# videosegmentation/video_segment

Hardware: AMD Instinct MI355X
Metric: over-segmented frames/sec at 1080p (higher is better)
Workload: dtype f32

## Files before the change

### include/vsg.h

```cpp
#ifndef VSG_H_
#define VSG_H_

#include <stddef.h>
#include <stdint.h>

#ifdef __cplusplus
extern "C" {
#endif

#define VSG_OK 0
#define VSG_ERR_INVALID -1
#define VSG_ERR_DEVICE -2
#define VSG_ERR_STATE -3
#define VSG_ERR_INTERNAL -4

#define VSG_MEM_HOST 0
#define VSG_MEM_DEVICE 1

typedef struct vsg_stream vsg_stream;
typedef struct vsg_graph vsg_graph;

typedef struct vsg_options {
  int presmoothing;
  float frac_min_region_size;
  int chunk_size;
  float chunk_overlap_ratio;
  int num_constraint_frames;
  int enforce_n4_connectivity;
  int enforce_spatial_connectedness;
  int color_distance;
  int device;
  int two_stage_oversegment;
  int compute_vectorization;
} vsg_options;

typedef struct vsg_timings {
  float preprocess_ms;
  float edges_ms;
  float sort_ms;
  float merge_ms;
  float readout_ms;
  float host_post_ms;
  int64_t edges_total;
  int64_t edges_active;
  int64_t merges;
  int64_t preprocess_launches;
  int64_t edge_launches;
  float wave_kernel_ms;
  int64_t wave_kernel_launches;
  int64_t wave_kernel_edges;
  float filter_kernel_ms;
  int64_t filter_kernel_launches;
  float spine_kernel_ms;
  int64_t spine_kernel_launches;
  int64_t spine_kernel_edges;
} vsg_timings;

typedef struct vsg_diagnostics {
  double segment_wall_ms;
  double prepare_ms;
  double constrained_merge_ms;
  int64_t stages;
  int64_t optimistic_stages, rollbacks;
  int64_t slab_growths;
  double slab_growth_ms;
  int64_t spine_pool_growths;
  double spine_pool_growth_ms;
  int64_t runtime_mallocs;
  double runtime_malloc_ms;
  int64_t runtime_frees;
  double runtime_free_ms;
  int64_t cache_hits;
  int64_t device_syncs;
  double device_sync_ms;
  int64_t mail_waits;
  double mail_wait_ms;
  double mail_wait_longest_ms;
  int mail_mode;
} vsg_diagnostics;

typedef struct vsg_merge_paths {
  int64_t hub_stages;
  int64_t hub_absorbed;
  int64_t hub_cuts;
  int64_t hub_cuts_in_groups;
  int64_t hub_parts_in_later_bucket;
  int64_t spine_side_cuts;
  int64_t hub_retries;
  int64_t hub_reasons[6];
  int64_t hub_exclusion_reruns;
  int64_t hub_off_reruns;
  int64_t group_halvings;
  int64_t conservative_replays;
} vsg_merge_paths;

typedef struct vsg_spine_paths {
  int64_t replays;
  int64_t components;
  int64_t nested_replays;
  int64_t deepest_level;
  int64_t forest_rounds;
  int64_t forest_rounds_ahead;
  int64_t forest_compactions_ahead;
  int64_t forest_compactions_sync;
  int64_t forest_lists_refused;
  int64_t ranked_by_sampling;
  int64_t ranked_plain;
  int64_t rank_sampling_refused;
  int64_t jump_loops_ended_early;
  int64_t streamed_passes;
  int64_t streamed_refused;
  int64_t pool_fallbacks[4];
  int64_t top_level_fallbacks;
  int64_t nested_fallbacks;
  int64_t assumption_reruns;
  int64_t limit_bucket_moves;
  int64_t low_bucket_failures[2];
  int64_t low_bucket_skips[2];
  int64_t zero_pool_flips;
  int64_t windows_run;
  int64_t rle_stages;
  int64_t wide_launches;
  int64_t group_stages;
  int64_t sorts_hand;
  int64_t sorts_library;
} vsg_spine_paths;

typedef struct vsg_boundary_paths {
  int64_t halo_planes_in_pool;
} vsg_boundary_paths;

typedef struct vsg_memory_stats {
  int64_t bytes_in_use;
  int64_t bytes_in_use_peak;
  int64_t bytes_cached;
  int64_t limit_bytes;
  int64_t runtime_mallocs, runtime_frees, cache_hits, device_syncs;
  double runtime_malloc_ms, runtime_free_ms, device_sync_ms;
} vsg_memory_stats;
int vsg_device_memory_stats(int device, vsg_memory_stats* out);
int vsg_device_memory_trim(int device);
int vsg_device_memory_limit(int device, int64_t bytes);

const char* vsg_last_error(void);
int vsg_version(void);
void vsg_default_options(vsg_options* o);
int vsg_device_count(void);

int vsg_vectorize_id_image(const int32_t* ids, int width, int height, const uint8_t** data,
                           size_t* len);

int vsg_stream_create(const vsg_options* o, int width, int height, vsg_stream** out);
void vsg_stream_destroy(vsg_stream* s);
int vsg_stream_process_frame(vsg_stream* s, int flush, const uint8_t* bgr, size_t stride,
                             const float* flow, int has_flow_stream, int mem, int* num_results);
int vsg_stream_chunk_size(const vsg_stream* s);
int vsg_stream_result_bytes(vsg_stream* s, int i, const uint8_t** data, size_t* len);
int vsg_stream_result_id_image(vsg_stream* s, int i, int32_t* out);
int vsg_stream_last_merge_stats(const vsg_stream* s, int64_t* forced_regular_small);
int vsg_stream_keep_node_states(vsg_stream* s, int on);
int vsg_stream_last_node_states(const vsg_stream* s, int64_t* n, const int32_t** root, const float** mean,
                                const int32_t** size, const int32_t** constraint, const uint8_t** flags);
int vsg_stream_last_timings(const vsg_stream* s, vsg_timings* t);
int vsg_stream_last_diagnostics(const vsg_stream* s, vsg_diagnostics* d);
int vsg_stream_last_merge_paths(const vsg_stream* s, vsg_merge_paths* out);
int vsg_stream_last_spine_paths(const vsg_stream* s, vsg_spine_paths* out);
int vsg_stream_last_boundary_paths(const vsg_stream* s, vsg_boundary_paths* out);
int vsg_stream_last_smoothed(vsg_stream* s, float* out);

int vsg_stream_export_halo(vsg_stream* s, const int32_t** dev_labels_virtual,
                           const int32_t** dev_labels_constrained, int64_t scalars[4]);
int vsg_stream_import_halo(vsg_stream* s, const int32_t* labels_virtual,
                           const int32_t* labels_constrained, int mem, const int64_t scalars[4]);

int vsg_stream_expect_halo(vsg_stream* s);
int vsg_stream_restart(vsg_stream* s);

typedef struct vsg_chain vsg_chain;
int vsg_chain_create(int rank, int world, const char* id_file, uint64_t nonce, int device,
                     vsg_chain** out);
void vsg_chain_destroy(vsg_chain* c);
int vsg_chain_info(const vsg_chain* c, int* rank, int* world);
int vsg_chain_send_halo(vsg_chain* c, vsg_stream* from, int dst);
int vsg_chain_recv_halo(vsg_chain* c, vsg_stream* into, int src);
int vsg_chain_exchange_halo(vsg_chain* c, vsg_stream* from, int dst, vsg_stream* into, int src);

typedef struct vsg_regionseg vsg_regionseg;
typedef struct vsg_regionseg_options {
  int min_region_num;
  int max_region_num;
  float level_cutoff_fraction;
  float small_region_penalizer;
  int luminance_bins;
  int color_bins;
  int flow_bins;
  int chunk_set_size;
  int chunk_set_overlap;
  int constraint_chunks;
  int use_appearance;
  int use_flow;
  int use_size_penalizer;
  int compute_vectorization;
  int save_descriptors;
} vsg_regionseg_options;
void vsg_regionseg_default_options(vsg_regionseg_options* o);
int vsg_regionseg_create(const vsg_regionseg_options* o, int width, int height, vsg_regionseg** out);
void vsg_regionseg_destroy(vsg_regionseg* r);
int vsg_regionseg_process_frame(vsg_regionseg* r, int flush, const uint8_t* seg_desc, size_t seg_len,
                             const uint8_t* bgr, size_t stride, const float* flow, int* num_results);
int vsg_regionseg_result_bytes(vsg_regionseg* r, int i, const uint8_t** data, size_t* len);
int vsg_bgr_to_lab(const uint8_t* bgr, size_t stride, int width, int height, uint8_t* lab);

int vsg_graph_create(int width, int height, int max_frames, int l1, int device, vsg_graph** out);
void vsg_graph_destroy(vsg_graph* g);
int vsg_graph_add_frame_bgr(vsg_graph* g, const uint8_t* bgr, size_t stride, int presmoothing,
                            const int32_t* constraint_ids, int mem);
int vsg_graph_add_frame_features(vsg_graph* g, const float* feat, const int32_t* constraint_ids,
                                 int mem);
int vsg_graph_add_virtual_frame(vsg_graph* g, const int32_t* constraint_ids, int mem);
int vsg_graph_add_temporal(vsg_graph* g, const float* flow, int is_virtual, int mem);
int vsg_graph_finish_building(vsg_graph* g);
int vsg_graph_segment_spatially(vsg_graph* g);
int vsg_graph_segment(vsg_graph* g, int min_region_size, int force_constraints);
int vsg_graph_obtain_results(vsg_graph* g, int use_flows, int enforce_n4,
                             int enforce_spatial_connectedness);
int vsg_graph_num_frames(const vsg_graph* g);
int vsg_graph_num_regions(const vsg_graph* g);
int64_t vsg_graph_num_neighbor_links(const vsg_graph* g);
int vsg_graph_region_sizes(const vsg_graph* g, int32_t* sizes, int32_t* constrained_ids);
int vsg_graph_index_image(const vsg_graph* g, int t, int32_t* out);
typedef struct vsg_region {
  int32_t index, size, constrained_id, first_frame, last_frame;
} vsg_region;
typedef struct vsg_interval {
  int32_t region_index, y, left_x, right_x;
} vsg_interval;
int vsg_graph_get_regions(vsg_graph* g, const vsg_region** regions, size_t* num_regions,
                          const int32_t** nbr_csr_ptr, const int32_t** nbr_csr_idx);
int vsg_graph_get_intervals(vsg_graph* g, int frame, const vsg_interval** intervals, size_t* n);
int vsg_graph_smoothed(vsg_graph* g, int t, float* out );
int vsg_graph_spatial_buckets(vsg_graph* g, int t, uint16_t* out );
int vsg_graph_temporal_buckets(vsg_graph* g, int t, uint16_t* out , int32_t* prev_idx);
int vsg_graph_node_roots(vsg_graph* g, int32_t* out);
int vsg_graph_node_states(vsg_graph* g, int32_t* root, float* mean, int32_t* size, int32_t* constraint,
                          uint8_t* flags);
int vsg_graph_merge_stats(const vsg_graph* g, int64_t* forced_regular_small);
int vsg_graph_timings(const vsg_graph* g, vsg_timings* t);
int vsg_graph_diagnostics(const vsg_graph* g, vsg_diagnostics* d);
int vsg_graph_merge_paths(const vsg_graph* g, vsg_merge_paths* out);
int vsg_graph_spine_paths(const vsg_graph* g, vsg_spine_paths* out);

int vsg_debug_sort_pairs(const uint32_t* keys, const uint32_t* values, int n, int end_bit,
                         uint32_t* keys_out, uint32_t* values_out, int device);
int vsg_debug_sort_pairs_timed(const uint32_t* keys, const uint32_t* values, int n, int end_bit,
                               uint32_t* keys_out, uint32_t* values_out, int device, int impl, int reps,
                               double* avg_us);
int vsg_debug_exclusive_sum(const int32_t* in, int n, int32_t* out, int64_t* total);
int vsg_debug_runs_of_sorted_keys(const uint32_t* keys, int n, int32_t* seg_off, int32_t* seg_cnt,
                                  int32_t* num_runs);

#ifdef __cplusplus
}
#endif
#endif
```

### video_segment_amd/_lib.py

```python
import ctypes as C
import os
import subprocess

_HERE = os.path.dirname(os.path.abspath(__file__))
CSRC_DIR = os.path.join(_HERE, "csrc")
LIB_PATH = os.path.join(_HERE, "lib", "libvsg_hip.so")

VSG_OK = 0
VSG_ERR_INVALID, VSG_ERR_DEVICE, VSG_ERR_STATE, VSG_ERR_INTERNAL = -1, -2, -3, -4
VSG_MEM_HOST = 0
VSG_MEM_DEVICE = 1


class VsgOptions(C.Structure):
    _fields_ = [
        ("presmoothing", C.c_int),
        ("frac_min_region_size", C.c_float),
        ("chunk_size", C.c_int),
        ("chunk_overlap_ratio", C.c_float),
        ("num_constraint_frames", C.c_int),
        ("enforce_n4_connectivity", C.c_int),
        ("enforce_spatial_connectedness", C.c_int),
        ("color_distance", C.c_int),
        ("device", C.c_int),
        ("two_stage_oversegment", C.c_int),
        ("compute_vectorization", C.c_int),
    ]


class VsgTimings(C.Structure):
    _fields_ = [
        ("preprocess_ms", C.c_float),
        ("edges_ms", C.c_float),
        ("sort_ms", C.c_float),
        ("merge_ms", C.c_float),
        ("readout_ms", C.c_float),
        ("host_post_ms", C.c_float),
        ("edges_total", C.c_int64),
        ("edges_active", C.c_int64),
        ("merges", C.c_int64),
        ("preprocess_launches", C.c_int64),
        ("edge_launches", C.c_int64),
        ("wave_kernel_ms", C.c_float),
        ("wave_kernel_launches", C.c_int64),
        ("wave_kernel_edges", C.c_int64),
        ("filter_kernel_ms", C.c_float),
        ("filter_kernel_launches", C.c_int64),
        ("spine_kernel_ms", C.c_float),
        ("spine_kernel_launches", C.c_int64),
        ("spine_kernel_edges", C.c_int64),
    ]


class VsgDiagnostics(C.Structure):
    _fields_ = [
        ("segment_wall_ms", C.c_double), ("prepare_ms", C.c_double), ("constrained_merge_ms", C.c_double),
        ("stages", C.c_int64), ("optimistic_stages", C.c_int64), ("rollbacks", C.c_int64),
        ("slab_growths", C.c_int64), ("slab_growth_ms", C.c_double),
        ("spine_pool_growths", C.c_int64), ("spine_pool_growth_ms", C.c_double),
        ("runtime_mallocs", C.c_int64), ("runtime_malloc_ms", C.c_double),
        ("runtime_frees", C.c_int64), ("runtime_free_ms", C.c_double),
        ("cache_hits", C.c_int64), ("device_syncs", C.c_int64), ("device_sync_ms", C.c_double),
        ("mail_waits", C.c_int64), ("mail_wait_ms", C.c_double), ("mail_wait_longest_ms", C.c_double),
        ("mail_mode", C.c_int),
    ]

    def as_dict(self):
        return {k: getattr(self, k) for k, _ in self._fields_}


class VsgMergePaths(C.Structure):
    _fields_ = [
        ("hub_stages", C.c_int64), ("hub_absorbed", C.c_int64),
        ("hub_cuts", C.c_int64), ("hub_cuts_in_groups", C.c_int64), ("hub_parts_in_later_bucket", C.c_int64),
        ("spine_side_cuts", C.c_int64),
        ("hub_retries", C.c_int64), ("hub_reasons", C.c_int64 * 6),
        ("hub_exclusion_reruns", C.c_int64), ("hub_off_reruns", C.c_int64),
        ("group_halvings", C.c_int64), ("conservative_replays", C.c_int64),
    ]

    def as_dict(self):
        return {k: (list(getattr(self, k)) if k == "hub_reasons" else getattr(self, k)) for k, _ in self._fields_}


class VsgSpinePaths(C.Structure):
    _fields_ = [
        ("replays", C.c_int64), ("components", C.c_int64), ("nested_replays", C.c_int64),
        ("deepest_level", C.c_int64),
        ("forest_rounds", C.c_int64), ("forest_rounds_ahead", C.c_int64), ("forest_compactions_ahead", C.c_int64),
        ("forest_compactions_sync", C.c_int64), ("forest_lists_refused", C.c_int64),
        ("ranked_by_sampling", C.c_int64), ("ranked_plain", C.c_int64), ("rank_sampling_refused", C.c_int64),
        ("jump_loops_ended_early", C.c_int64), ("streamed_passes", C.c_int64), ("streamed_refused", C.c_int64),
        ("pool_fallbacks", C.c_int64 * 4), ("top_level_fallbacks", C.c_int64), ("nested_fallbacks", C.c_int64),
        ("assumption_reruns", C.c_int64), ("limit_bucket_moves", C.c_int64),
        ("low_bucket_failures", C.c_int64 * 2), ("low_bucket_skips", C.c_int64 * 2),
        ("zero_pool_flips", C.c_int64),
        ("windows_run", C.c_int64), ("rle_stages", C.c_int64), ("wide_launches", C.c_int64),
        ("group_stages", C.c_int64), ("sorts_hand", C.c_int64), ("sorts_library", C.c_int64),
    ]

    def as_dict(self):
        return {k: (list(getattr(self, k)) if issubclass(t, C.Array) else getattr(self, k)) for k, t in self._fields_}


class VsgBoundaryPaths(C.Structure):
    _fields_ = [
        ("halo_planes_in_pool", C.c_int64),
    ]

    def as_dict(self):
        return {k: getattr(self, k) for k, _ in self._fields_}


class VsgMemoryStats(C.Structure):
    _fields_ = [
        ("bytes_in_use", C.c_int64), ("bytes_in_use_peak", C.c_int64), ("bytes_cached", C.c_int64),
        ("limit_bytes", C.c_int64),
        ("runtime_mallocs", C.c_int64), ("runtime_frees", C.c_int64), ("cache_hits", C.c_int64),
        ("device_syncs", C.c_int64),
        ("runtime_malloc_ms", C.c_double), ("runtime_free_ms", C.c_double), ("device_sync_ms", C.c_double),
    ]

    def as_dict(self):
        return {k: getattr(self, k) for k, _ in self._fields_}


class VsgRegionOptions(C.Structure):
    _fields_ = [
        ("min_region_num", C.c_int), ("max_region_num", C.c_int),
        ("level_cutoff_fraction", C.c_float), ("small_region_penalizer", C.c_float),
        ("luminance_bins", C.c_int), ("color_bins", C.c_int), ("flow_bins", C.c_int),
        ("chunk_set_size", C.c_int), ("chunk_set_overlap", C.c_int), ("constraint_chunks", C.c_int),
        ("use_appearance", C.c_int), ("use_flow", C.c_int), ("use_size_penalizer", C.c_int),
        ("compute_vectorization", C.c_int), ("save_descriptors", C.c_int),
    ]


EXPORTED_SYMBOLS = [
    "vsg_last_error", "vsg_version", "vsg_default_options", "vsg_device_count",
    "vsg_device_memory_stats", "vsg_device_memory_trim", "vsg_device_memory_limit",
    "vsg_vectorize_id_image",
    "vsg_stream_create", "vsg_stream_destroy", "vsg_stream_process_frame", "vsg_stream_chunk_size",
    "vsg_stream_result_bytes", "vsg_stream_result_id_image", "vsg_stream_last_merge_stats",
    "vsg_stream_keep_node_states", "vsg_stream_last_node_states",
    "vsg_stream_last_timings", "vsg_stream_last_diagnostics", "vsg_stream_last_merge_paths", "vsg_stream_last_spine_paths",
    "vsg_stream_last_boundary_paths",
    "vsg_stream_last_smoothed", "vsg_stream_export_halo",
    "vsg_stream_import_halo", "vsg_stream_expect_halo", "vsg_stream_restart",
    "vsg_chain_create", "vsg_chain_destroy", "vsg_chain_info", "vsg_chain_send_halo",
    "vsg_chain_recv_halo", "vsg_chain_exchange_halo",
    "vsg_regionseg_default_options", "vsg_regionseg_create", "vsg_regionseg_destroy", "vsg_regionseg_process_frame",
    "vsg_regionseg_result_bytes", "vsg_bgr_to_lab",
    "vsg_graph_create", "vsg_graph_destroy", "vsg_graph_add_frame_bgr",
    "vsg_graph_add_frame_features", "vsg_graph_add_virtual_frame", "vsg_graph_add_temporal",
    "vsg_graph_finish_building", "vsg_graph_segment_spatially", "vsg_graph_segment", "vsg_graph_obtain_results",
    "vsg_graph_num_frames", "vsg_graph_num_regions", "vsg_graph_num_neighbor_links",
    "vsg_graph_region_sizes", "vsg_graph_index_image", "vsg_graph_get_regions",
    "vsg_graph_get_intervals", "vsg_graph_smoothed",
    "vsg_graph_spatial_buckets", "vsg_graph_temporal_buckets", "vsg_graph_node_roots",
    "vsg_graph_node_states",
    "vsg_graph_merge_stats", "vsg_graph_timings", "vsg_graph_diagnostics", "vsg_graph_merge_paths",
    "vsg_graph_spine_paths",
    "vsg_debug_sort_pairs", "vsg_debug_sort_pairs_timed", "vsg_debug_exclusive_sum", "vsg_debug_runs_of_sorted_keys",
]


def build(force=False):
    subprocess.check_call(["make", "-C", CSRC_DIR, "-j8", "-s"])
    return LIB_PATH


_lib = None


def lib():
    global _lib
    if _lib is not None:
        return _lib
    if not os.path.exists(LIB_PATH):
        raise RuntimeError(
            "libvsg_hip.so is missing (%s): build the HIP extension first; there is no fallback "
            "path" % LIB_PATH)
    try:
        import torch
    except ImportError:
        pass
    L = C.CDLL(LIB_PATH)
    vp = C.c_void_p
    L.vsg_last_error.restype = C.c_char_p
    L.vsg_version.restype = C.c_int
    L.vsg_default_options.argtypes = [C.POINTER(VsgOptions)]
    L.vsg_device_count.restype = C.c_int
    L.vsg_device_memory_stats.argtypes = [C.c_int, C.POINTER(VsgMemoryStats)]
    L.vsg_device_memory_trim.argtypes = [C.c_int]
    L.vsg_device_memory_limit.argtypes = [C.c_int, C.c_int64]
    L.vsg_vectorize_id_image.argtypes = [vp, C.c_int, C.c_int, C.POINTER(vp), C.POINTER(C.c_size_t)]
    L.vsg_stream_create.argtypes = [C.POINTER(VsgOptions), C.c_int, C.c_int, C.POINTER(vp)]
    L.vsg_stream_destroy.argtypes = [vp]
    L.vsg_stream_process_frame.argtypes = [vp, C.c_int, vp, C.c_size_t, vp, C.c_int, C.c_int,
                                           C.POINTER(C.c_int)]
    L.vsg_stream_chunk_size.argtypes = [vp]
    L.vsg_stream_result_bytes.argtypes = [vp, C.c_int, C.POINTER(vp), C.POINTER(C.c_size_t)]
    L.vsg_stream_result_id_image.argtypes = [vp, C.c_int, vp]
    L.vsg_stream_last_merge_stats.argtypes = [vp, vp]
    L.vsg_stream_keep_node_states.argtypes = [vp, C.c_int]
    L.vsg_stream_last_node_states.argtypes = [vp, C.POINTER(C.c_int64)] + [C.POINTER(vp)] * 5
    L.vsg_stream_last_timings.argtypes = [vp, C.POINTER(VsgTimings)]
    L.vsg_stream_last_diagnostics.argtypes = [vp, C.POINTER(VsgDiagnostics)]
    L.vsg_stream_last_merge_paths.argtypes = [vp, C.POINTER(VsgMergePaths)]
    L.vsg_stream_last_spine_paths.argtypes = [vp, C.POINTER(VsgSpinePaths)]
    L.vsg_stream_last_boundary_paths.argtypes = [vp, C.POINTER(VsgBoundaryPaths)]
    L.vsg_stream_last_smoothed.argtypes = [vp, vp]
    L.vsg_stream_export_halo.argtypes = [vp, C.POINTER(vp), C.POINTER(vp), vp]
    L.vsg_stream_import_halo.argtypes = [vp, vp, vp, C.c_int, vp]
    L.vsg_stream_expect_halo.argtypes = [vp]
    L.vsg_stream_restart.argtypes = [vp]
    L.vsg_chain_create.argtypes = [C.c_int, C.c_int, C.c_char_p, C.c_uint64, C.c_int, C.POINTER(vp)]
    L.vsg_chain_info.argtypes = [vp, C.POINTER(C.c_int), C.POINTER(C.c_int)]
    L.vsg_chain_exchange_halo.argtypes = [vp, vp, C.c_int, vp, C.c_int]
    L.vsg_chain_destroy.argtypes = [vp]
    L.vsg_chain_send_halo.argtypes = [vp, vp, C.c_int]
    L.vsg_chain_recv_halo.argtypes = [vp, vp, C.c_int]
    L.vsg_regionseg_default_options.argtypes = [C.POINTER(VsgRegionOptions)]
    L.vsg_regionseg_create.argtypes = [C.POINTER(VsgRegionOptions), C.c_int, C.c_int, C.POINTER(vp)]
    L.vsg_regionseg_destroy.argtypes = [vp]
    L.vsg_regionseg_process_frame.argtypes = [vp, C.c_int, vp, C.c_size_t, vp, C.c_size_t, vp, C.POINTER(C.c_int)]
    L.vsg_regionseg_result_bytes.argtypes = [vp, C.c_int, C.POINTER(vp), C.POINTER(C.c_size_t)]
    L.vsg_bgr_to_lab.argtypes = [vp, C.c_size_t, C.c_int, C.c_int, vp]
    L.vsg_debug_sort_pairs.argtypes = [vp, vp, C.c_int, C.c_int, vp, vp, C.c_int]
    L.vsg_debug_sort_pairs_timed.argtypes = [vp, vp, C.c_int, C.c_int, vp, vp, C.c_int, C.c_int, C.c_int,
                                             C.POINTER(C.c_double)]
    L.vsg_graph_create.argtypes = [C.c_int, C.c_int, C.c_int, C.c_int, C.c_int, C.POINTER(vp)]
    L.vsg_graph_destroy.argtypes = [vp]
    L.vsg_graph_add_frame_bgr.argtypes = [vp, vp, C.c_size_t, C.c_int, vp, C.c_int]
    L.vsg_graph_add_frame_features.argtypes = [vp, vp, vp, C.c_int]
    L.vsg_graph_add_virtual_frame.argtypes = [vp, vp, C.c_int]
    L.vsg_graph_add_temporal.argtypes = [vp, vp, C.c_int, C.c_int]
    L.vsg_graph_finish_building.argtypes = [vp]
    L.vsg_graph_segment_spatially.argtypes = [vp]
    L.vsg_graph_segment.argtypes = [vp, C.c_int, C.c_int]
    L.vsg_graph_obtain_results.argtypes = [vp, C.c_int, C.c_int, C.c_int]
    L.vsg_graph_num_frames.argtypes = [vp]
    L.vsg_graph_num_regions.argtypes = [vp]
    L.vsg_graph_num_neighbor_links.argtypes = [vp]
    L.vsg_graph_num_neighbor_links.restype = C.c_int64
    L.vsg_graph_region_sizes.argtypes = [vp, vp, vp]
    L.vsg_graph_index_image.argtypes = [vp, C.c_int, vp]
    L.vsg_graph_get_regions.argtypes = [vp, C.POINTER(vp), C.POINTER(C.c_size_t), C.POINTER(vp),
                                        C.POINTER(vp)]
    L.vsg_graph_get_intervals.argtypes = [vp, C.c_int, C.POINTER(vp), C.POINTER(C.c_size_t)]
    L.vsg_graph_smoothed.argtypes = [vp, C.c_int, vp]
    L.vsg_graph_spatial_buckets.argtypes = [vp, C.c_int, vp]
    L.vsg_graph_temporal_buckets.argtypes = [vp, C.c_int, vp, vp]
    L.vsg_graph_node_roots.argtypes = [vp, vp]
    L.vsg_graph_node_states.argtypes = [vp, vp, vp, vp, vp, vp]
    L.vsg_graph_merge_stats.argtypes = [vp, vp]
    L.vsg_graph_timings.argtypes = [vp, C.POINTER(VsgTimings)]
    L.vsg_graph_diagnostics.argtypes = [vp, C.POINTER(VsgDiagnostics)]
    L.vsg_graph_merge_paths.argtypes = [vp, C.POINTER(VsgMergePaths)]
    L.vsg_graph_spine_paths.argtypes = [vp, C.POINTER(VsgSpinePaths)]
    L.vsg_debug_exclusive_sum.argtypes = [vp, C.c_int, vp, C.POINTER(C.c_int64)]
    L.vsg_debug_runs_of_sorted_keys.argtypes = [vp, C.c_int, vp, vp, C.POINTER(C.c_int32)]
    _lib = L
    return L


class VsgError(RuntimeError):

    def __init__(self, msg, code=None):
        super().__init__(msg)
        self.code = code


def memory_stats(device=-1):
    st = VsgMemoryStats()
    check(lib().vsg_device_memory_stats(device, C.byref(st)))
    return st.as_dict()


def memory_trim(device=-1):
    check(lib().vsg_device_memory_trim(device))


def memory_limit(nbytes, device=-1):
    check(lib().vsg_device_memory_limit(device, int(nbytes)))


def check(rc):
    if rc != VSG_OK:
        raise VsgError("vsg error %d: %s" % (rc, lib().vsg_last_error().decode()), rc)
```

### video_segment_amd/csrc/capi.cpp

```cpp
#include <algorithm>
#include <cstring>
#include <memory>
#include <string>
#include <vector>

#include <rccl/rccl.h>

#include <chrono>
#include <cstdio>
#include <fstream>
#include <thread>

#include "../../include/vsg.h"
#include "region_segmentation.h"
#include "scan_device.h"
#include "stream.h"

namespace {

thread_local std::string g_last_error;

template <class F>
int Guard(F&& f) {
  try {
// ... 235 lines not shown
        runs.emplace_back(row[x], vsg::Interval{y, x, x2});
        x = x2 + 1;
      }
    }
    std::stable_sort(runs.begin(), runs.end(),
                     [](const std::pair<int32_t, vsg::Interval>& a,
                        const std::pair<int32_t, vsg::Interval>& b) { return a.first < b.first; });
    vsg::SegDesc d;
    d.frame_width = width;
    d.frame_height = height;
    for (const auto& r : runs) {
      if (d.regions.empty() || d.regions.back().id != r.first) {
        d.regions.emplace_back();
        d.regions.back().id = r.first;
      }
      d.regions.back().raster.push_back(r.second);
    }
    for (auto& r : d.regions) vsg::MomentsFromRaster(r.raster, &r.moments);
    vsg::ComputeFrameVectorization(&d);
    wire = vsg::EncodeSegDesc(d);
    *data = reinterpret_cast<const uint8_t*>(wire.data());
    *len = wire.size();
  });
}

static void RequireFrameSize(int width, int height) {
  VSG_REQUIRE(width >= 2 && width <= vsg::kMaxFrameWidth && height >= 1 && height <= vsg::kMaxFrameHeight,
              VSG_ERR_INVALID,
              "unsupported frame size " + std::to_string(width) + "x" + std::to_string(height) +
                  ": width has to be in [2, " + std::to_string(vsg::kMaxFrameWidth) +
                  "], height in [1, " + std::to_string(vsg::kMaxFrameHeight) + "]");
}

int vsg_stream_create(const vsg_options* o, int width, int height, vsg_stream** out) {
  return Guard([&] {
    VSG_REQUIRE(o && out, VSG_ERR_INVALID, "null argument");
    RequireFrameSize(width, height);
    RequireDevice(o->device);
    std::unique_ptr<vsg_stream> s(new vsg_stream);
    s->device = ResolveDevice(o->device);
    DeviceGuard dg(s->device);
    vsg_options opts = *o;
    opts.device = s->device;
    s->impl.reset(new vsg::DenseSegmentationHip(opts, width, height));
    *out = s.release();
  });
}

void vsg_stream_destroy(vsg_stream* s) {
  if (!s) return;
  (void)Guard([&] {
    DeviceGuard dg(s->device);
    s->impl.reset();
  });
  delete s;
}

int vsg_stream_process_frame(vsg_stream* s, int flush, const uint8_t* bgr, size_t stride,
                             const float* flow, int has_flow_stream, int mem, int* num_results) {
  return Guard([&] {
    VSG_REQUIRE(s && num_results, VSG_ERR_INVALID, "null argument");
    DeviceGuard dg(s->device);
    *num_results = s->impl->ProcessFrame(flush != 0, bgr, stride, flow, has_flow_stream != 0, mem);
  });
}

int vsg_stream_chunk_size(const vsg_stream* s) { return s ? s->impl->ChunkSize() : VSG_ERR_INVALID; }

int vsg_stream_result_bytes(vsg_stream* s, int i, const uint8_t** data, size_t* len) {
  return Guard([&] {
    VSG_REQUIRE(s && data && len, VSG_ERR_INVALID, "null argument");
    DeviceGuard dg(s->device);
    VSG_REQUIRE(i >= 0 && i < s->impl->num_results(), VSG_ERR_INVALID, "result index");
    const std::string& b = s->impl->result_bytes(i);
    *data = reinterpret_cast<const uint8_t*>(b.data());
    *len = b.size();
  });
}

int vsg_stream_result_id_image(vsg_stream* s, int i, int32_t* out) {
  return Guard([&] {
    VSG_REQUIRE(s && out, VSG_ERR_INVALID, "null argument");
    DeviceGuard dg(s->device);
    VSG_REQUIRE(i >= 0 && i < s->impl->num_results(), VSG_ERR_INVALID, "result index");
    const size_t n = (size_t)s->impl->W() * s->impl->H();
    for (size_t k = 0; k < n; ++k) out[k] = -1;
    vsg::RenderIdImage(s->impl->result(i), s->impl->W(), out);
  });
}

int vsg_stream_last_merge_stats(const vsg_stream* s, int64_t* st) {
  return Guard([&] {
    VSG_REQUIRE(s && st, VSG_ERR_INVALID, "null argument");
    DeviceGuard dg(s->device);
    s->impl->last_merge_stats(st);
  });
}

int vsg_stream_keep_node_states(vsg_stream* s, int on) {
  return Guard([&] {
    VSG_REQUIRE(s, VSG_ERR_INVALID, "null argument");
    s->impl->keep_node_states(on != 0);
  });
}

int vsg_stream_last_node_states(const vsg_stream* s, int64_t* n, const int32_t** root, const float** mean,
                                const int32_t** size, const int32_t** constraint, const uint8_t** flags) {
  return Guard([&] {
    VSG_REQUIRE(s && n && root && mean && size && constraint && flags, VSG_ERR_INVALID, "null argument");
    const auto& st = s->impl->last_node_states();
    VSG_REQUIRE(!st.root.empty(), VSG_ERR_STATE, "no chunk has been segmented with keeping on");
    *n = (int64_t)st.root.size();
    *root = st.root.data();
    *mean = st.mean.data();
    *size = st.size.data();
    *constraint = st.constraint.data();
    *flags = st.flags.data();
  });
}

int vsg_stream_last_timings(const vsg_stream* s, vsg_timings* t) {
  return Guard([&] {
    VSG_REQUIRE(s && t, VSG_ERR_INVALID, "null argument");
    DeviceGuard dg(s->device);
    *t = s->impl->last_timings();
  });
}

int vsg_stream_last_diagnostics(const vsg_stream* s, vsg_diagnostics* d) {
  return Guard([&] {
    VSG_REQUIRE(s && d, VSG_ERR_INVALID, "null argument");
    FillDiagnostics(s->impl->last_graph_timings(), d);
  });
}

int vsg_stream_last_merge_paths(const vsg_stream* s, vsg_merge_paths* out) {
  return Guard([&] {
    VSG_REQUIRE(s && out, VSG_ERR_INVALID, "null argument");
    FillMergePaths(s->impl->last_graph_timings().paths, out);
  });
}

int vsg_stream_last_spine_paths(const vsg_stream* s, vsg_spine_paths* out) {
  return Guard([&] {
    VSG_REQUIRE(s && out, VSG_ERR_INVALID, "null argument");
    FillSpinePaths(s->impl->last_graph_timings().spine_paths, out);
  });
}

int vsg_stream_last_boundary_paths(const vsg_stream* s, vsg_boundary_paths* out) {
  return Guard([&] {
    VSG_REQUIRE(s && out, VSG_ERR_INVALID, "null argument");
    *out = s->impl->last_boundary_paths();
  });
}

int vsg_stream_last_smoothed(vsg_stream* s, float* out) {
  return Guard([&] {
    VSG_REQUIRE(s && out, VSG_ERR_INVALID, "null argument");
    DeviceGuard dg(s->device);
    s->impl->CopyLastSmoothed(out);
  });
}

int vsg_stream_export_halo(vsg_stream* s, const int32_t** virt, const int32_t** cons,
                           int64_t scalars[4]) {
  return Guard([&] {
    VSG_REQUIRE(s && virt && cons && scalars, VSG_ERR_INVALID, "null argument");
    DeviceGuard dg(s->device);
    s->impl->ExportHalo(virt, cons, scalars);
  });
}

int vsg_stream_expect_halo(vsg_stream* s) {
  return Guard([&] {
    VSG_REQUIRE(s, VSG_ERR_INVALID, "null argument");
    DeviceGuard dg(s->device);
    s->impl->ExpectHalo();
  });
}

int vsg_stream_restart(vsg_stream* s) {
  return Guard([&] {
    VSG_REQUIRE(s, VSG_ERR_INVALID, "null argument");
    DeviceGuard dg(s->device);
    s->impl->Restart();
  });
}

int vsg_stream_import_halo(vsg_stream* s, const int32_t* virt, const int32_t* cons, int mem,
                           const int64_t scalars[4]) {
  return Guard([&] {
    VSG_REQUIRE(s && virt && cons && scalars, VSG_ERR_INVALID, "null argument");
    DeviceGuard dg(s->device);
    s->impl->ImportHalo(virt, cons, mem, scalars);
  });
}

}

#define VSG_NCCL(call)                                                                      \
  do {                                                                                      \
    ncclResult_t r_ = (call);                                                               \
    if (r_ != ncclSuccess) {                                                                \
      vsg::Throw(VSG_ERR_DEVICE, std::string("RCCL: ") + ncclGetErrorString(r_) + " in " #call); \
    }                                                                                       \
  } while (0)

struct vsg_chain {
  int rank = 0, world = 1, device = 0;
  ncclComm_t comm = nullptr;
  hipStream_t stream = nullptr;
  vsg::DevBuf<int32_t> send_staging, recv_staging;
};

namespace {

struct ChainIdFile {
  char magic[8];
  uint64_t nonce;
  ncclUniqueId id;
};
const char kChainMagic[8] = {'V', 'S', 'G', 'C', 'H', 'A', 'I', 'N'};

}

extern "C" {

int vsg_chain_create(int rank, int world, const char* id_file, uint64_t nonce, int device,
                     vsg_chain** out) {
  return Guard([&] {
    VSG_REQUIRE(out && id_file && world >= 1 && rank >= 0 && rank < world, VSG_ERR_INVALID,
                "bad argument");
    RequireDevice(device);
    std::unique_ptr<vsg_chain> c(new vsg_chain);
    c->rank = rank;
    c->world = world;
    c->device = ResolveDevice(device);
    DeviceGuard dg(c->device);
    ChainIdFile rec;
    const std::string path(id_file);
    if (rank == 0) {
      (void)std::remove(path.c_str());
      std::memcpy(rec.magic, kChainMagic, sizeof(rec.magic));
      rec.nonce = nonce;
      VSG_NCCL(ncclGetUniqueId(&rec.id));
      const std::string tmp = path + ".tmp";
      {
        std::ofstream f(tmp.c_str(), std::ios::binary | std::ios::trunc);
        f.write(reinterpret_cast<const char*>(&rec), sizeof(rec));
        VSG_REQUIRE(f.good(), VSG_ERR_INVALID, "cannot write the communicator id file");
      }
      VSG_REQUIRE(std::rename(tmp.c_str(), path.c_str()) == 0, VSG_ERR_INVALID,
                  "cannot publish the communicator id file");
    } else {
      bool got = false;
      for (int attempt = 0; attempt < 1200 && !got; ++attempt) {
        std::ifstream f(path.c_str(), std::ios::binary);
        if (f.good()) {
          f.read(reinterpret_cast<char*>(&rec), sizeof(rec));
          got = f.gcount() == (std::streamsize)sizeof(rec) &&
                std::memcmp(rec.magic, kChainMagic, sizeof(rec.magic)) == 0 && rec.nonce == nonce;
        }
        if (!got) std::this_thread::sleep_for(std::chrono::milliseconds(100));
      }
      VSG_REQUIRE(got, VSG_ERR_STATE,
                  "timed out waiting for the communicator id file of this run (nonce mismatch or "
                  "rank 0 never started)");
    }
    VSG_NCCL(ncclCommInitRank(&c->comm, world, rec.id, rank));
    if (rank == 0) (void)std::remove(path.c_str());
    VSG_HIP(hipStreamCreateWithFlags(&c->stream, hipStreamNonBlocking));
    *out = c.release();
  });
}

void vsg_chain_destroy(vsg_chain* c) {
  if (!c) return;
  (void)Guard([&] {
    DeviceGuard dg(c->device);
    if (c->stream) (void)hipStreamSynchronize(c->stream);
    if (c->comm) (void)ncclCommDestroy(c->comm);
    if (c->stream) (void)hipStreamDestroy(c->stream);
    c->send_staging.release();
    c->recv_staging.release();
  });
  delete c;
}

int vsg_chain_info(const vsg_chain* c, int* rank, int* world) {
  return Guard([&] {
    VSG_REQUIRE(c && rank && world, VSG_ERR_INVALID, "null argument");
    DeviceGuard dg(c->device);
    VSG_NCCL(ncclCommUserRank(c->comm, rank));
    VSG_NCCL(ncclCommCount(c->comm, world));
  });
}

int vsg_chain_exchange_halo(vsg_chain* c, vsg_stream* from, int dst, vsg_stream* into, int src) {
  return Guard([&] {
    VSG_REQUIRE(c && (from || into), VSG_ERR_INVALID, "bad argument");
    VSG_REQUIRE(!from || (dst >= 0 && dst < c->world), VSG_ERR_INVALID, "destination rank");
    VSG_REQUIRE(!into || (src >= 0 && src < c->world), VSG_ERR_INVALID, "source rank");
    VSG_REQUIRE(!from || dst != c->rank || (into && src == c->rank), VSG_ERR_INVALID,
                "a send to the own rank needs the matching receive in the same call");
    VSG_REQUIRE(!into || src != c->rank || (from && dst == c->rank), VSG_ERR_INVALID,
// ... 156 lines not shown
    if (n == 0) return;
    vsg::DevBuf<uint32_t> k((size_t)n), v((size_t)n), ko((size_t)n), vo((size_t)n);
    vsg::DevBuf<uint8_t> temp(vsg::SortPairsU32TempBytes(n));
    hipStream_t s = nullptr;
    VSG_HIP(hipStreamCreateWithFlags(&s, hipStreamNonBlocking));
    hipEvent_t e0 = nullptr, e1 = nullptr;
    struct Owner {
      hipStream_t& s;
      hipEvent_t &e0, &e1;
      ~Owner() {
        if (e0) (void)hipEventDestroy(e0);
        if (e1) (void)hipEventDestroy(e1);
        (void)hipStreamDestroy(s);
      }
    } owner{s, e0, e1};
    VSG_HIP(hipEventCreate(&e0));
    VSG_HIP(hipEventCreate(&e1));
    VSG_HIP(hipMemcpyAsync(k.get(), keys, (size_t)n * 4, hipMemcpyHostToDevice, s));
    VSG_HIP(hipMemcpyAsync(v.get(), values, (size_t)n * 4, hipMemcpyHostToDevice, s));
    auto sort = impl == 1 ? vsg::SortPairsU32Hand : impl == 2 ? vsg::SortPairsU32Lib : vsg::SortPairsU32;
    sort(temp.get(), temp.size(), k.get(), ko.get(), v.get(), vo.get(), n, end_bit, s);
    VSG_HIP(hipEventRecord(e0, s));
    for (int r = 0; r < reps; ++r) sort(temp.get(), temp.size(), k.get(), ko.get(), v.get(), vo.get(), n, end_bit, s);
    VSG_HIP(hipEventRecord(e1, s));
    VSG_HIP(hipMemcpyAsync(keys_out, ko.get(), (size_t)n * 4, hipMemcpyDeviceToHost, s));
    VSG_HIP(hipMemcpyAsync(values_out, vo.get(), (size_t)n * 4, hipMemcpyDeviceToHost, s));
    VSG_HIP(hipStreamSynchronize(s));
    float ms = 0;
    VSG_HIP(hipEventElapsedTime(&ms, e0, e1));
    if (avg_us) *avg_us = (double)ms * 1e3 / reps;
  });
}

int vsg_debug_sort_pairs(const uint32_t* keys, const uint32_t* values, int n, int end_bit,
                         uint32_t* keys_out, uint32_t* values_out, int device) {
  return vsg_debug_sort_pairs_timed(keys, values, n, end_bit, keys_out, values_out, device, 0, 1, nullptr);
}

namespace {
struct DebugStream {
  hipStream_t s = nullptr;
  DebugStream() { VSG_HIP(hipStreamCreateWithFlags(&s, hipStreamNonBlocking)); }
  ~DebugStream() { (void)hipStreamDestroy(s); }
};
}

int vsg_debug_exclusive_sum(const int32_t* in, int n, int32_t* out, int64_t* total) {
  return Guard([&] {
    VSG_REQUIRE(in && out && total && n >= 0, VSG_ERR_INVALID, "bad argument");
    RequireDevice(-1);
    if (n == 0) return;
    vsg::DevBuf<int32_t> d_in((size_t)n), d_out(in == out ? (size_t)1 : (size_t)n), sums(vsg::kScanMaxTiles), d_total(1);
    int32_t* o = in == out ? d_in.get() : d_out.get();
    DebugStream st;
    VSG_HIP(hipMemcpyAsync(d_in.get(), in, (size_t)n * 4, hipMemcpyHostToDevice, st.s));
    vsg::DebugExclusiveSum(vsg::ScanScratch{sums.get(), nullptr}, d_in.get(), o, n, d_total.get(), st.s);
    int32_t t = 0;
    VSG_HIP(hipMemcpyAsync(out, o, (size_t)n * 4, hipMemcpyDeviceToHost, st.s));
    VSG_HIP(hipMemcpyAsync(&t, d_total.get(), 4, hipMemcpyDeviceToHost, st.s));
    VSG_HIP(hipStreamSynchronize(st.s));
    *total = t;
  });
}

int vsg_debug_runs_of_sorted_keys(const uint32_t* keys, int n, int32_t* seg_off, int32_t* seg_cnt,
                                  int32_t* num_runs) {
  return Guard([&] {
    VSG_REQUIRE(keys && seg_off && seg_cnt && num_runs && n >= 0, VSG_ERR_INVALID, "bad argument");
    RequireDevice(-1);
    if (n == 0) return;
    vsg::DevBuf<uint32_t> d_keys((size_t)n);
    vsg::DevBuf<int32_t> d_off((size_t)n), d_cnt((size_t)n), sums(vsg::kScanMaxTiles), d_runs(1);
    DebugStream st;
    VSG_HIP(hipMemcpyAsync(d_keys.get(), keys, (size_t)n * 4, hipMemcpyHostToDevice, st.s));
    VSG_HIP(hipMemcpyAsync(d_off.get(), seg_off, (size_t)n * 4, hipMemcpyHostToDevice, st.s));
    VSG_HIP(hipMemcpyAsync(d_cnt.get(), seg_cnt, (size_t)n * 4, hipMemcpyHostToDevice, st.s));
    vsg::RunsOfSortedKeys(vsg::ScanScratch{sums.get(), nullptr}, d_keys.get(), n, d_off.get(), d_cnt.get(), d_runs.get(),
                          st.s);
    VSG_HIP(hipMemcpyAsync(seg_off, d_off.get(), (size_t)n * 4, hipMemcpyDeviceToHost, st.s));
    VSG_HIP(hipMemcpyAsync(seg_cnt, d_cnt.get(), (size_t)n * 4, hipMemcpyDeviceToHost, st.s));
    VSG_HIP(hipMemcpyAsync(num_runs, d_runs.get(), 4, hipMemcpyDeviceToHost, st.s));
    VSG_HIP(hipStreamSynchronize(st.s));
  });
}

int vsg_graph_create(int width, int height, int max_frames, int l1, int device, vsg_graph** out) {
  return Guard([&] {
    VSG_REQUIRE(out, VSG_ERR_INVALID, "null argument");
    RequireFrameSize(width, height);
    RequireDevice(device);
    std::unique_ptr<vsg_graph> g(new vsg_graph);
    g->device = ResolveDevice(device);
    DeviceGuard dg(g->device);
    g->W = width;
    g->H = height;
    g->wh = (size_t)width * height;
    VSG_HIP(hipStreamCreateWithFlags(&g->stream, hipStreamNonBlocking));
    g->g.reset(new vsg::DenseGraphHip(width, height, max_frames, l1 != 0, g->stream));
    g->pre.reset(new vsg::Preprocessor(width, height, g->stream));
    std::memset(&g->timings, 0, sizeof(g->timings));
    *out = g.release();
  });
}

void vsg_graph_destroy(vsg_graph* g) {
  if (!g) return;
  (void)Guard([&] {
    DeviceGuard dg(g->device);
    if (g->stream) (void)hipStreamSynchronize(g->stream);
    vsg::QuiesceGuard quiesce;
    quiesce.Begin();
    g->g.reset();
    g->pre.reset();
    g->feats.clear();
    g->staging_bgr.release();
    g->staging_f32.release();
    g->staging_ids.release();
    g->flows_dev.clear();
    if (g->stream) (void)hipStreamDestroy(g->stream);
    g->stream = nullptr;
  });
  delete g;
}

static const int32_t* StageIds(vsg_graph* g, const int32_t* ids, int mem) {
  if (!ids) return nullptr;
  if (mem == VSG_MEM_DEVICE) return ids;
  g->staging_ids.ensure(g->wh);
  VSG_HIP(hipMemcpyAsync(g->staging_ids.get(), ids, g->wh * sizeof(int32_t), hipMemcpyHostToDevice,
                         g->stream));
  return g->staging_ids.get();
}

int vsg_graph_add_frame_bgr(vsg_graph* g, const uint8_t* bgr, size_t stride, int presmoothing,
                            const int32_t* constraint_ids, int mem) {
  return Guard([&] {
    VSG_REQUIRE(g && bgr, VSG_ERR_INVALID, "null argument");
    DeviceGuard dg(g->device);
    VSG_REQUIRE(stride >= (size_t)g->W * 3, VSG_ERR_INVALID, "stride smaller than a row");
    const uint8_t* dev = bgr;
    if (mem == VSG_MEM_HOST) {
      g->staging_bgr.ensure(stride * (size_t)g->H);
      VSG_HIP(hipMemcpyAsync(g->staging_bgr.get(), bgr,
                             stride * (size_t)(g->H - 1) + (size_t)g->W * 3, hipMemcpyHostToDevice,
                             g->stream));
      dev = g->staging_bgr.get();
    }
    auto feat = std::make_shared<vsg::DevBuf<float>>(3 * g->wh);
    g->pre->Run(dev, stride, presmoothing, feat->get());
    g->timings.preprocess_ms += g->pre->last_ms();
    g->timings.preprocess_launches += 1;
    const int32_t* ids = StageIds(g, constraint_ids, mem);
    g->g->AddFrame(feat->get(), ids);
    VSG_HIP(hipStreamSynchronize(g->stream));
    g->feats.push_back(feat);
    g->flows_dev.push_back(nullptr);
  });
}

int vsg_graph_add_frame_features(vsg_graph* g, const float* feat_in, const int32_t* constraint_ids,
                                 int mem) {
  return Guard([&] {
    VSG_REQUIRE(g && feat_in, VSG_ERR_INVALID, "null argument");
    DeviceGuard dg(g->device);
    const float* src = feat_in;
    if (mem == VSG_MEM_HOST) {
      g->staging_f32.ensure(3 * g->wh);
      VSG_HIP(hipMemcpyAsync(g->staging_f32.get(), feat_in, 3 * g->wh * sizeof(float),
                             hipMemcpyHostToDevice, g->stream));
      src = g->staging_f32.get();
    }
    auto feat = std::make_shared<vsg::DevBuf<float>>(3 * g->wh);
    vsg::LaunchInterleavedToPlanar(src, g->wh, feat->get(), g->stream);
    const int32_t* ids = StageIds(g, constraint_ids, mem);
    g->g->AddFrame(feat->get(), ids);
    VSG_HIP(hipStreamSynchronize(g->stream));
    g->feats.push_back(feat);
    g->flows_dev.push_back(nullptr);
  });
}

int vsg_graph_add_virtual_frame(vsg_graph* g, const int32_t* constraint_ids, int mem) {
  return Guard([&] {
    VSG_REQUIRE(g && constraint_ids, VSG_ERR_INVALID, "null argument");
    DeviceGuard dg(g->device);
    std::vector<int32_t> host(g->wh);
    if (mem == VSG_MEM_HOST) {
      std::memcpy(host.data(), constraint_ids, g->wh * sizeof(int32_t));
    } else {
      VSG_HIP(hipMemcpy(host.data(), constraint_ids, g->wh * sizeof(int32_t), hipMemcpyDeviceToHost));
    }
    int max_label = 0;
    for (int32_t v : host) max_label = std::max(max_label, v + 1);
    const int32_t* ids = StageIds(g, constraint_ids, mem);
    g->g->AddVirtualFrame(ids, std::max(max_label, 1));
    VSG_HIP(hipStreamSynchronize(g->stream));
    g->feats.push_back(nullptr);
    g->flows_dev.push_back(nullptr);
  });
}

int vsg_graph_add_temporal(vsg_graph* g, const float* flow, int is_virtual, int mem) {
  return Guard([&] {
    VSG_REQUIRE(g, VSG_ERR_INVALID, "null argument");
    DeviceGuard dg(g->device);
    const int nf = g->g->num_frames();
    VSG_REQUIRE(nf >= 2, VSG_ERR_STATE, "temporal edges need two slices");
    const float* fdev = nullptr;
    if (flow) {
      auto fd = std::make_shared<vsg::DevBuf<float>>(2 * g->wh);
      VSG_HIP(hipMemcpyAsync(fd->get(), flow, 2 * g->wh * sizeof(float),
                             mem == VSG_MEM_HOST ? hipMemcpyHostToDevice : hipMemcpyDeviceToDevice,
                             g->stream));
      g->flows_dev[nf - 1] = fd;
      fdev = fd->get();
    }
    const float* cur = g->feats[nf - 1] ? g->feats[nf - 1]->get() : nullptr;
    const float* prev = g->feats[nf - 2] ? g->feats[nf - 2]->get() : nullptr;
    VSG_REQUIRE(is_virtual || (cur && prev), VSG_ERR_STATE, "real temporal edges need two real slices");
    g->g->AddTemporal(cur, prev, fdev, is_virtual != 0);
    VSG_HIP(hipStreamSynchronize(g->stream));
  });
}

int vsg_graph_finish_building(vsg_graph* g) {
  return Guard([&] {
    VSG_REQUIRE(g, VSG_ERR_INVALID, "null argument");
    DeviceGuard dg(g->device);
    g->g->FinishBuilding();
  });
}

int vsg_graph_segment_spatially(vsg_graph* g) {
  return Guard([&] {
    VSG_REQUIRE(g, VSG_ERR_INVALID, "null argument");
    DeviceGuard dg(g->device);
    g->g->SegmentSpatially();
  });
}

int vsg_graph_segment(vsg_graph* g, int min_region_size, int force_constraints) {
  return Guard([&] {
    VSG_REQUIRE(g, VSG_ERR_INVALID, "null argument");
    DeviceGuard dg(g->device);
    g->g->Segment(min_region_size, force_constraints != 0);
  });
}

int vsg_graph_obtain_results(vsg_graph* g, int use_flows, int enforce_n4,
                             int enforce_spatial_connectedness) {
  return Guard([&] {
    VSG_REQUIRE(g, VSG_ERR_INVALID, "null argument");
    DeviceGuard dg(g->device);
    std::vector<const float*> flows;
    if (use_flows) {
      for (auto& f : g->flows_dev) flows.push_back(f ? f->get() : nullptr);
    }
    g->g->ObtainResults(use_flows ? &flows : nullptr, enforce_n4 != 0,
                        enforce_spatial_connectedness != 0);
  });
}

int vsg_graph_num_frames(const vsg_graph* g) { return g ? g->g->num_frames() : VSG_ERR_INVALID; }
int vsg_graph_num_regions(const vsg_graph* g) {
  return g ? (int)g->g->regions().size() : VSG_ERR_INVALID;
}
int64_t vsg_graph_num_neighbor_links(const vsg_graph* g) {
  if (!g) return VSG_ERR_INVALID;
  int64_t n = 0;
  for (const auto& r : g->g->regions()) n += (int64_t)r.neighbors.size();
  return n;
}

int vsg_graph_region_sizes(const vsg_graph* g, int32_t* sizes, int32_t* constrained_ids) {
  return Guard([&] {
    VSG_REQUIRE(g && sizes && constrained_ids, VSG_ERR_INVALID, "null argument");
    DeviceGuard dg(g->device);
    const auto& regs = g->g->regions();
    for (size_t i = 0; i < regs.size(); ++i) {
      sizes[i] = regs[i].size;
      constrained_ids[i] = regs[i].constrained_id;
    }
  });
}

int vsg_graph_index_image(const vsg_graph* g, int t, int32_t* out) {
  return Guard([&] {
    VSG_REQUIRE(g && out, VSG_ERR_INVALID, "null argument");
    DeviceGuard dg(g->device);
    for (size_t k = 0; k < g->wh; ++k) out[k] = -1;
    for (const auto& r : g->g->regions()) {
      if (!r.has_raster) continue;
      for (const auto& sl : r.raster) {
        if (sl.frame != t) continue;
        for (const auto& iv : sl.raster) {
          for (int x = iv.lx; x <= iv.rx; ++x) out[(size_t)iv.y * g->W + x] = r.index;
        }
      }
    }
  });
}

int vsg_graph_get_regions(vsg_graph* g, const vsg_region** regions, size_t* num_regions,
                          const int32_t** nbr_csr_ptr, const int32_t** nbr_csr_idx) {
  return Guard([&] {
    VSG_REQUIRE(g && regions && num_regions && nbr_csr_ptr && nbr_csr_idx, VSG_ERR_INVALID,
                "null argument");
    const auto& regs = g->g->regions();
    g->out_regions.resize(regs.size());
    g->out_nbr_ptr.assign(regs.size() + 1, 0);
    g->out_nbr_idx.clear();
    for (size_t i = 0; i < regs.size(); ++i) {
      const vsg::RegionInfo& r = regs[i];
      VSG_REQUIRE(r.index == (int)i, VSG_ERR_INTERNAL, "region table out of order");
      vsg_region& o = g->out_regions[i];
      o.index = r.index;
      o.size = r.size;
      o.constrained_id = r.constrained_id;
      const bool has = r.has_raster && !r.raster.empty();
      o.first_frame = has ? r.raster.front().frame : -1;
      o.last_frame = has ? r.raster.back().frame : -1;
      g->out_nbr_idx.insert(g->out_nbr_idx.end(), r.neighbors.begin(), r.neighbors.end());
      g->out_nbr_ptr[i + 1] = (int32_t)g->out_nbr_idx.size();
    }
    if (g->out_nbr_idx.empty()) g->out_nbr_idx.push_back(0);
    *regions = g->out_regions.data();
    *num_regions = regs.size();
    *nbr_csr_ptr = g->out_nbr_ptr.data();
// ... 127 lines not shown
```

### video_segment_amd/csrc/dense_graph.cpp

```cpp
#include "dense_graph.h"
#include "scan_device.h"

#include <algorithm>
#include <chrono>
#include <cmath>
#include <cstring>
#include <atomic>
#include <functional>
#include <thread>
#include <unordered_set>

namespace vsg {

namespace {
template <class T>
DevBuf<T>& Grow(DevBuf<T>& b, size_t n) {
  if (b.size() < n) b.alloc(n + n / 2 + 1024);
  return b;
}
double NowMs() {
  using clk = std::chrono::steady_clock;
  return std::chrono::duration<double, std::milli>(clk::now().time_since_epoch()).count();
}
template <class T>
void D2H(T* dst, const T* src, size_t n, hipStream_t s) {
  if (n == 0) return;
  VSG_HIP(hipMemcpyAsync(dst, src, n * sizeof(T), hipMemcpyDeviceToHost, s));
}
template <class T>
void H2D(T* dst, const T* src, size_t n, hipStream_t s) {
  if (n == 0) return;
  VSG_HIP(hipMemcpyAsync(dst, src, n * sizeof(T), hipMemcpyHostToDevice, s));
}
}

DenseGraphHip::DenseGraphHip(int W, int H, int max_frames, bool l1, hipStream_t stream)
    : W_(W), H_(H), capacity_frames_(max_frames), max_frames_(max_frames), l1_(l1),
      stream_(stream), wh_((size_t)W * H) {
  VSG_REQUIRE(W >= 2 && H >= 1 && W <= kMaxFrameWidth && H <= kMaxFrameHeight, -1, "unsupported frame size");
  VSG_REQUIRE(max_frames >= 1 && max_frames < 4096, -1, "unsupported number of frames");
  const size_t N = wh_ * (size_t)max_frames;
  VSG_REQUIRE(N * 9 < (size_t)0xFFFFFFFFu, -1, "graph too large for 32-bit edge positions");
  parent_.alloc(N);
  desc_sz_.alloc(N);
  cons_.alloc(N);
  flags_.alloc(N);
  hub8_.alloc(N);
  cc_.alloc(N);
  label_uf_.alloc(N);
  label_img_.alloc(N);
  adjust_.alloc(N);
  lists_.resize(2 * max_frames - 1);
  list_desc_dev_.alloc(lists_.size());
  list_slot_base_dev_.alloc(lists_.size() + 1);
  const size_t total_slots = (size_t)(4 * max_frames + 9 * (max_frames - 1)) * wh_;
  kept_all_.alloc(total_slots);
  bucket_base_dev_.alloc((size_t)(kNumBuckets + 1) * (lists_.size() + 1));
  keys_tmp_.alloc(9 * wh_ + 8);
  hist_tmp_.alloc(EdgeSortHistInts(wh_));
  hist_sums_.alloc(EdgeSortSumInts(wh_) + 1);
  scalars_.alloc(32);
  stats_.alloc(96);
  hub_excl_.alloc(kHubListInts);
  VSG_HIP(hipMemsetAsync(hub_excl_.get(), 0, 4 * sizeof(int32_t), stream_));
  {
    const int slots = 256;
    const size_t list_cap = 8192;
    const size_t bytes = (size_t)slots * kMailValues * sizeof(unsigned long long) + list_cap * sizeof(int32_t);
    mail_mem_ = CacheAlloc(bytes, kCacheMappedCoherent);
    std::memset(mail_mem_, 0, bytes);
    void* dev = nullptr;
    VSG_HIP(hipHostGetDevicePointer(&dev, mail_mem_, 0));
    mail_.host = static_cast<volatile unsigned long long*>(mail_mem_);
    mail_.dev = static_cast<unsigned long long*>(dev);
    mail_.slots = slots;
    mail_.list_host = reinterpret_cast<volatile int32_t*>(static_cast<char*>(mail_mem_) +
                                                          (size_t)slots * kMailValues * sizeof(unsigned long long));
    mail_.list_dev = reinterpret_cast<int32_t*>(static_cast<char*>(dev) +
                                                (size_t)slots * kMailValues * sizeof(unsigned long long));
    mail_.list_cap = (int)list_cap;
    zero_pool_mem_.alloc(1 << 20);
    zero_pool_.base = zero_pool_mem_.get();
    zero_pool_.cap = zero_pool_mem_.size();
    if (const char* e = getenv("VSG_ZERO_POOL")) {
      zero_pool_.cap = std::min<size_t>(zero_pool_.cap, std::max<size_t>((size_t)atoll(e), 4096) + kZeroArenaInts);
    }
  }
  VSG_HIP(hipStreamCreateWithFlags(&aux_stream_, hipStreamNonBlocking));
  VSG_HIP(hipStreamCreateWithFlags(&aux2_stream_, hipStreamNonBlocking));
  VSG_HIP(hipEventCreateWithFlags(&aux_fork_, hipEventDisableTiming));
  VSG_HIP(hipEventCreateWithFlags(&aux_join_, hipEventDisableTiming));

  scan_sums_.alloc(kScanMaxTiles);
  Reset(max_frames);
  MailRegisterGraph(1);
}

DenseGraphHip::~DenseGraphHip() {
  quiesce_.Begin();
  MailRegisterGraph(-1);
  for (hipEvent_t e : ev_pool_) (void)hipEventDestroy(e);
  if (aux_fork_) (void)hipEventDestroy(aux_fork_);
  if (aux_join_) (void)hipEventDestroy(aux_join_);
  if (aux_stream_) (void)hipStreamDestroy(aux_stream_);
  if (aux2_stream_) (void)hipStreamDestroy(aux2_stream_);
  if (mail_mem_) CacheFree(mail_mem_);
}

void DenseGraphHip::Reset(int max_frames) {
  VSG_REQUIRE(max_frames >= 1 && max_frames <= capacity_frames_, -1, "max_frames above capacity");
  max_frames_ = max_frames;
  num_frames_ = 0;
  has_constraints_ = false;
  virtual_slices_.clear();
  flattened_ = false;
  spatial_pass_done_ = false;
  halo_pending_ = false;
  deferred_virtual_slice_ = deferred_constrained_slice_ = -1;
  for (auto& lb : lists_) lb.used = false;
  regions_.clear();
  key_to_region_.clear();
  key_size_override_.clear();
  next_region_index_ = 0;
  timings_ = GraphTimings();
}

void DenseGraphHip::ForgetLearned() {
  spine_limit_bucket_ = 0x7fffffff;
  spine_limit_age_ = 0;
  for (int b = 0; b < 2; ++b) {
    spine_low_fails_[b] = spine_low_cooldown_[b] = spine_low_cost_age_[b] = 0;
    spine_low_cost_fail_[b] = spine_low_cost_skip_[b] = 0;
  }
  wave_target_active_ = kNoWindowTarget;
  window_target_.clear();
  hub_bucket_pause_.clear();
  window_target_age_ = 0;
  last_density_ = 1.0;
}

void DenseGraphHip::SortList(ListBuf& lb, int per_px) {
  const int n = (int)(per_px * wh_);
  lb.slots.ensure((size_t)n);
  lb.offsets.ensure(kBucketSlots);
  LaunchBucketSort(keys_tmp_.get(), wh_, per_px, hist_tmp_.get(), hist_sums_.get(),
                   lb.offsets.get(), lb.slots.get(), stream_);
  lb.n = n;
  lb.used = true;
}

void DenseGraphHip::AddFrame(const float* feat, const int32_t* cons_dev) {
  VSG_REQUIRE(num_frames_ < max_frames_, -1, "more frames than max_frames (CHECK_LE)");
  const int t = num_frames_;
  const int base = (int)(wh_ * t);
  LaunchInitNodes(feat, wh_, base, cons_dev, nodes(), stream_);
  ListBuf& lb = lists_[2 * t];
  lb.type = 0;
  lb.base_a = base;
  lb.base_b = base;
  LaunchSpatialKeys(feat, W_, H_, l1_ ? 1 : 0, keys_tmp_.get(), hist_tmp_.get(), stream_);
  SortList(lb, 4);
  if (cons_dev) has_constraints_ = true;
  ++num_frames_;
}

void DenseGraphHip::AddVirtualFrame(const int32_t* ids_dev, int max_label) {
  VSG_REQUIRE(num_frames_ < max_frames_, -1, "more frames than max_frames (CHECK_LE)");
  VSG_REQUIRE(max_label >= 1, -1, "max_label must be positive");
  const int t = num_frames_;
  first_label_scratch_.ensure((size_t)max_label);
  LaunchInitVirtualNodes(ids_dev, wh_, (int)(wh_ * t), max_label, first_label_scratch_.get(),
                         nodes(), stream_);
  virtual_slices_.push_back(t);
  has_constraints_ = true;
  ++num_frames_;
}

void DenseGraphHip::AddVirtualFrameDeferred() {
  VSG_REQUIRE(num_frames_ < max_frames_, -1, "more frames than max_frames (CHECK_LE)");
  deferred_virtual_slice_ = num_frames_;
  deferred_constrained_slice_ = num_frames_ + 1;
  virtual_slices_.push_back(num_frames_);
  has_constraints_ = true;
  halo_pending_ = true;
  ++num_frames_;
}

void DenseGraphHip::SetHaloLabels(const int32_t* virtual_ids_dev, const int32_t* constrained_ids_dev,
                                  int max_label) {
  VSG_REQUIRE(halo_pending_, -3, "no deferred virtual slice");
  VSG_REQUIRE(num_frames_ > deferred_constrained_slice_, -3,
              "the constrained slice has to be added before its labels");
  VSG_REQUIRE(max_label >= 1, -1, "max_label must be positive");
  first_label_scratch_.ensure((size_t)max_label);
  LaunchInitVirtualNodes(virtual_ids_dev, wh_, (int)(wh_ * deferred_virtual_slice_), max_label,
                         first_label_scratch_.get(), nodes(), stream_);
  VSG_HIP(hipMemcpyAsync(cons_.get() + wh_ * (size_t)deferred_constrained_slice_, constrained_ids_dev,
                         wh_ * sizeof(int32_t), hipMemcpyDeviceToDevice, stream_));
  halo_pending_ = false;
}

void DenseGraphHip::AddTemporal(const float* cur, const float* prev, const float* flow,
                                bool is_virtual) {
  VSG_REQUIRE(num_frames_ >= 2, -3, "temporal edges need two slices");
  const int t = num_frames_ - 1;
  ListBuf& lb = lists_[2 * t - 1];
  lb.type = 1;
  lb.base_a = (int)(wh_ * t);
  lb.base_b = (int)(wh_ * (t - 1));
  lb.prev_idx.ensure(wh_);
  LaunchTemporalKeys(cur, prev, flow, W_, H_, l1_ ? 1 : 0, is_virtual ? 1 : 0, keys_tmp_.get(),
                     lb.prev_idx.get(), hist_tmp_.get(), stream_);
  SortList(lb, 9);
}

void DenseGraphHip::FinishBuilding() { VSG_HIP(hipStreamSynchronize(stream_)); }

void DenseGraphHip::EnsureScratch(size_t n) {
  if (n <= scratch_edges_) return;
  n = n + n / 8 + 1024;
  e_ra_.alloc(n);
  e_rb_.alloc(n);
  e_gpos_.alloc(n);
  filter_masks_.alloc(3 * (4 * ((n + 255) / 256) + 4));
  block_cnt_.alloc((n + 255) / 256 + 2);
  block_off_.alloc((n + 255) / 256 + 2);
  scratch_edges_ = n;
}

void DenseGraphHip::EnsureActiveScratch(size_t n) {
  if (n <= scratch_active_) return;
  n = std::max(n + n / 8 + 1024, scratch_active_ + scratch_active_ / 2);
  size_t bytes = 0;
  auto carve = [&bytes](size_t elems, size_t elem_size) {
    const size_t at = bytes;
    bytes += (elems * elem_size + 255) & ~(size_t)255;
    return at;
  };
  const size_t o_e_active = carve(n, 4), o_e_apos = carve(n, 4), o_a_ra = carve(n, 4), o_a_rb = carve(n, 4),
               o_a_gpos = carve(n, 4), o_a_comp = carve(n, 4), o_a_idx = carve(n, 4), o_s_comp = carve(n, 4),
               o_s_idx = carve(n, 4), o_seg_key = carve(n, 4), o_seg_cnt = carve(n, 4), o_seg_off = carve(n, 4),
               o_lead_pos = carve(n, 4), o_l_ra = carve(n, 4), o_l_rb = carve(n, 4), o_l_gpos = carve(n, 4),
               o_bk_ds = carve(2 * n, sizeof(float4)), o_bk_cons = carve(2 * n, 4), o_bk_flags = carve(2 * n, 1);
  scratch_active_ = 0;
  act_ = ActiveArrays();
  active_slab_.alloc(bytes);
  uint8_t* b = active_slab_.get();
  act_.e_active = reinterpret_cast<int32_t*>(b + o_e_active);
  act_.e_apos = reinterpret_cast<int32_t*>(b + o_e_apos);
  act_.a_ra = reinterpret_cast<int32_t*>(b + o_a_ra);
  act_.a_rb = reinterpret_cast<int32_t*>(b + o_a_rb);
  act_.a_gpos = reinterpret_cast<uint32_t*>(b + o_a_gpos);
  act_.a_comp = reinterpret_cast<uint32_t*>(b + o_a_comp);
  act_.a_idx = reinterpret_cast<uint32_t*>(b + o_a_idx);
  act_.s_comp = reinterpret_cast<uint32_t*>(b + o_s_comp);
  act_.s_idx = reinterpret_cast<uint32_t*>(b + o_s_idx);
  act_.seg_key = reinterpret_cast<uint32_t*>(b + o_seg_key);
  act_.seg_cnt = reinterpret_cast<int32_t*>(b + o_seg_cnt);
  act_.seg_off = reinterpret_cast<int32_t*>(b + o_seg_off);
  act_.lead_pos = reinterpret_cast<int32_t*>(b + o_lead_pos);
  act_.l_ra = reinterpret_cast<int32_t*>(b + o_l_ra);
  act_.l_rb = reinterpret_cast<int32_t*>(b + o_l_rb);
  act_.l_gpos = reinterpret_cast<uint32_t*>(b + o_l_gpos);
  act_.bk_ds = reinterpret_cast<float4*>(b + o_bk_ds);
  act_.bk_cons = reinterpret_cast<int32_t*>(b + o_bk_cons);
  act_.bk_flags = b + o_bk_flags;
  const size_t temp = SortPairsU32TempBytes((int)std::min<size_t>(2 * n, 0x7fffffff));
  if (temp > cub_temp_.size()) cub_temp_.alloc(temp);
  scratch_active_ = n;
}

void DenseGraphHip::RunStageDebug(int b, int w, int windows, int j0, int n, const MergeParams& P,
                                  int inert_mode, MergeScratch& S, bool debug_stages, StageInfo* info) {
  unsigned long long s0[96] = {0}, s1[96] = {0};
  double ts = 0;
  size_t ev0 = 0, evf0 = 0;
  if (debug_stages) {
    VSG_HIP(hipMemsetAsync(stats_.get() + 16, 0, 2 * sizeof(unsigned long long), stream_));
    VSG_HIP(hipMemsetAsync(stats_.get() + 48, 0, 16 * sizeof(unsigned long long), stream_));
    D2H(s0, stats_.get(), 96, stream_);
    VSG_HIP(hipStreamSynchronize(stream_));
    ts = NowMs();
    ev0 = ev_wave_.size();
    evf0 = ev_filter_.size();
  }
  RunBucketStage(b, j0, n, list_desc_dev_.get(), bucket_base_dev_.get(), list_slot_base_dev_.get(),
                 kept_all_.get(), nodes(), P, inert_mode, S, stream_, info);
  if (!debug_stages) return;
  D2H(s1, stats_.get(), 96, stream_);
  VSG_HIP(hipStreamSynchronize(stream_));
  const double te = NowMs();
  float wave_ms = 0;
  for (size_t k = ev0; k < ev_wave_.size(); ++k) {
    float ms = 0;
    VSG_HIP(hipEventElapsedTime(&ms, ev_pool_[ev_wave_[k].first], ev_pool_[ev_wave_[k].second]));
    wave_ms += ms;
  }
  float filter_ms = 0;
  for (size_t k = evf0; k < ev_filter_.size(); ++k) {
    float ms = 0;
    VSG_HIP(hipEventElapsedTime(&ms, ev_pool_[ev_filter_[k].first], ev_pool_[ev_filter_[k].second]));
    filter_ms += ms;
  }
  if (te - ts <= 1.0) return;
  std::fprintf(stderr, "[vsg] stage b=%d w=%d/%d n=%d wall %.2f ms filter %.2f ms workers %.2f ms | replayed %d components %d | "
               "wave edges %llu batches %llu rounds %llu nwin %llu chain %llu | max_seg %llu slowest %.2f Mcyc | "
               "cyc load %.0f M loop %.0f M wait %.0f M\n",
               b, w, windows, n, te - ts, filter_ms, wave_ms, info ? info->replayed : -1, info ? info->components : -1,
               s1[3] - s0[3], s1[7] - s0[7], s1[5] - s0[5], s1[4] - s0[4], s1[20] - s0[20],
               s1[17], s1[16] / 1e6, (s1[18] - s0[18]) / 1e6, (s1[19] - s0[19]) / 1e6,
               (s1[26] - s0[26]) / 1e6);
  std::fprintf(stderr, "[vsg]   largest: %.2f Mcyc batches %llu rounds %llu live %llu chain %llu nwin %llu | kcyc/batch: "
               "wait %.1f stage+table %.1f loop %.1f (reserve %.1f closure %.1f masks+generic %.1f chain %.1f) | cuts %llu kept %llu\n",
               s1[48] / 1e6, s1[49], s1[50], s1[51], s1[55], s1[56],
               s1[52] / 1e3 / std::max(1.0, (double)s1[49]), s1[53] / 1e3 / std::max(1.0, (double)s1[49]),
               s1[54] / 1e3 / std::max(1.0, (double)s1[49]), s1[57] / 1e3 / std::max(1.0, (double)s1[49]),
               s1[58] / 1e3 / std::max(1.0, (double)s1[49]), s1[59] / 1e3 / std::max(1.0, (double)s1[49]),
               s1[60] / 1e3 / std::max(1.0, (double)s1[49]), s1[61], s1[62]);
  std::fprintf(stderr, "[vsg]   chain ends (%llu): not owner %llu, flags %llu, constraint %llu, larger %llu, failed/mode %llu, "
               "hot small %llu, none %llu\n", s1[71] - s0[71], s1[64] - s0[64], s1[65] - s0[65], s1[66] - s0[66],
               s1[67] - s0[67], s1[68] - s0[68], s1[69] - s0[69], s1[70] - s0[70]);
}

void DenseGraphHip::SegmentLists(int min_region_size, bool force_constraints, int pass) {
  VSG_REQUIRE(num_frames_ >= 1, -3, "no frames");
  VSG_REQUIRE(!halo_pending_, -3, "the labels of the previous chunk have not been imported");
  min_region_size_ = min_region_size;
  const int L = (int)lists_.size();
  const size_t N = wh_ * (size_t)num_frames_;
  const double t_enter = NowMs();
  const ThreadAllocCounters alloc0 = ThreadAllocSnapshot();
  MailWaitResetLongest();
  const MailWaitCounters mail0 = MailWaitSnapshot();
  int64_t diag_stages = 0, diag_slab_growths = 0, diag_spine_growths = 0, diag_hub_stages = 0, diag_hub_absorbed = 0;
  double diag_slab_ms = 0, diag_spine_ms = 0;

  std::vector<ListDesc> desc(L);
  list_slot_base_.assign(L + 1, 0);
  uint32_t acc = 0;
  int64_t edges_total = 0;
  for (int l = 0; l < L; ++l) {
    ListBuf& lb = lists_[l];
    list_slot_base_[l] = acc;
    ListDesc d = {};
    if (lb.used) {
      d.slots = lb.slots.get();
      d.kept = kept_all_.get() + acc;
      d.prev_idx = lb.type == 1 ? lb.prev_idx.get() : nullptr;
      d.offsets = (pass == 1 && lb.type == 1) ? nullptr : lb.offsets.get();
      d.type = lb.type;
      d.base_a = lb.base_a;
      d.base_b = lb.base_b;
      d.n = lb.n;
      acc += (uint32_t)lb.n;
    }
    desc[l] = d;
  }
  list_slot_base_[L] = acc;
  H2D(list_desc_dev_.get(), desc.data(), (size_t)L, stream_);
  H2D(list_slot_base_dev_.get(), list_slot_base_.data(), (size_t)L + 1, stream_);
  if (pass == 2) {
    kept_spatial_pass_.ensure(kept_all_.size());
    VSG_HIP(hipMemcpyAsync(kept_spatial_pass_.get(), kept_all_.get(), acc, hipMemcpyDeviceToDevice,
                           stream_));
  }
  VSG_HIP(hipMemsetAsync(kept_all_.get(), 0, acc, stream_));
  LaunchBuildBucketTable(list_desc_dev_.get(), L, bucket_base_dev_.get(), stream_);
  bucket_base_host_.resize((size_t)(kNumBuckets + 1) * (L + 1));
  D2H(bucket_base_host_.data(), bucket_base_dev_.get(), bucket_base_host_.size(), stream_);
  VSG_HIP(hipMemsetAsync(stats_.get(), 0, 96 * sizeof(unsigned long long), stream_));
  VSG_HIP(hipMemsetAsync(zero_pool_.base, 0, zero_pool_.cap * sizeof(int32_t), stream_));
  zero_pool_.used = 0;
  zero_pool_.second_half = false;
  zero_pool_.arena_used = 0;
  LaunchInitIdentity(cc_.get(), N, stream_);
  VSG_HIP(hipStreamSynchronize(stream_));

  const bool group_buckets = !getenv("VSG_GROUP_BUCKETS") || atoi(getenv("VSG_GROUP_BUCKETS")) != 0;
  std::vector<int32_t> bucket_prefix(kNumBuckets + 2, 0);
  int first_plain = kNumBuckets;
  {
    const float scale = 2048.0f / (1.0f + 1e-6f);
    const float inv_scale = (float)(1.0 / (double)scale);
    const float force_w = l1_ ? 0.002f : 0.001f;
    for (int b = 0; b < kNumBuckets; ++b) {
      if (!((float)b * inv_scale < force_w)) {
        first_plain = b;
        break;
      }
    }
  }
  int64_t n_max = 0;
  for (int b = 0; b <= kNumBuckets; ++b) {
    const int tot = bucket_base_host_[(size_t)b * (L + 1) + L];
    edges_total += tot;
    bucket_prefix[b + 1] = bucket_prefix[b] + tot;
  }
  for (int b = 0; b < kNumBuckets; ++b) n_max = std::max<int64_t>(n_max, bucket_prefix[b + 1] - bucket_prefix[b]);
  VSG_REQUIRE(bucket_prefix[kNumBuckets] >= 0, -1, "too many edges");
  EnsureScratch((size_t)std::max<int64_t>(n_max, 1));
  if (const char* e = getenv("VSG_ACTIVE_CAP")) {
    EnsureActiveScratch((size_t)std::max(1, atoi(e)));
  } else {
    EnsureActiveScratch(std::min<size_t>((size_t)std::max<int64_t>(n_max, 1),
                                         std::max<size_t>((size_t)n_max / 6, (size_t)1 << 20)));
  }
  bucket_prefix_dev_.ensure(bucket_prefix.size());
  H2D(bucket_prefix_dev_.get(), bucket_prefix.data(), bucket_prefix.size(), stream_);

  MergeScratch S = {};
  auto bind_scratch = [this, &S]() {
    S.e_ra = e_ra_.get();
    S.e_rb = e_rb_.get();
    S.e_gpos = e_gpos_.get();
    S.e_active = act_.e_active;
    S.e_apos = act_.e_apos;
    S.a_ra = act_.a_ra;
    S.a_rb = act_.a_rb;
    S.a_gpos = act_.a_gpos;
    S.a_comp = act_.a_comp;
    S.a_idx = act_.a_idx;
    S.s_comp = act_.s_comp;
    S.s_idx = act_.s_idx;
    S.seg_key = act_.seg_key;
    S.seg_cnt = act_.seg_cnt;
    S.seg_off = act_.seg_off;
    S.lead_pos = act_.lead_pos;
    S.l_ra = act_.l_ra;
    S.l_rb = act_.l_rb;
    S.l_gpos = act_.l_gpos;
    S.bk_ds = act_.bk_ds;
    S.bk_cons = act_.bk_cons;
    S.bk_flags = act_.bk_flags;
    S.cub_temp = cub_temp_.get();
    S.cub_temp_bytes = cub_temp_.size();
    S.scan = ScanScratch{scan_sums_.get(), stream_};
    S.active_cap = (int)std::min<size_t>(scratch_active_, 0x7fffffff);
  };
  bind_scratch();
  S.grow_active = [this, bind_scratch, &diag_slab_growths, &diag_slab_ms](long long need) {
    const double tg0 = NowMs();
    VSG_HIP(hipStreamSynchronize(stream_));
    VSG_HIP(hipStreamSynchronize(aux_stream_));
    VSG_HIP(hipStreamSynchronize(aux2_stream_));
    const size_t before = scratch_active_;
    EnsureActiveScratch((size_t)need);
    bind_scratch();
    ++diag_slab_growths;
    diag_slab_ms += NowMs() - tg0;
    if (getenv("VSG_DEBUG_STATS")) {
      std::fprintf(stderr, "[vsg] stage scratch: %zu -> %zu active edges (needed %lld), %.2f ms\n", before,
                   scratch_active_, need, NowMs() - tg0);
    }
    return true;
  };
  S.num_active = scalars_.get();
  S.num_segs = scalars_.get() + 1;
  S.node_key_bits = 1;
  while (S.node_key_bits < 32 && ((size_t)1 << S.node_key_bits) < N) ++S.node_key_bits;
  {
    const size_t words = 4 * ((scratch_edges_ + 255) / 256) + 4;
    S.masks.active = filter_masks_.get();
    S.masks.settled = filter_masks_.get() + words;
    S.masks.tentative = filter_masks_.get() + 2 * words;
    S.masks.block_cnt = block_cnt_.get();
    S.block_off = block_off_.get();
  }
  S.force_rollback = getenv("VSG_FORCE_ROLLBACK") ? 1 : 0;
  S.small_seg = getenv("VSG_SMALL_SEG") ? std::max(1, atoi(getenv("VSG_SMALL_SEG"))) : 24;
  S.wide_min = getenv("VSG_WIDE_MIN") ? atoi(getenv("VSG_WIDE_MIN")) : 0;
  S.wide_waves = getenv("VSG_WIDE_WAVES") ? atoi(getenv("VSG_WIDE_WAVES")) : 4;
  S.chain_relax = getenv("VSG_CHAIN_RELAX") ? atoi(getenv("VSG_CHAIN_RELAX")) : 1;
  const int hubs_default = getenv("VSG_HUBS") ? atoi(getenv("VSG_HUBS")) : 1;
  S.hubs = hubs_default;
  S.hub_excl = hub_excl_.get();
  S.hub_max_splits = getenv("VSG_HUB_SPLITS") ? std::max(0, atoi(getenv("VSG_HUB_SPLITS"))) : kHubMaxSplits;
  S.hub_cut_min_work = getenv("VSG_CUT_MIN_WORK") ? atoi(getenv("VSG_CUT_MIN_WORK")) : 0;
  S.hub_cut_ratio = getenv("VSG_CUT_RATIO") ? std::max(0, atoi(getenv("VSG_CUT_RATIO"))) : 1500;
  S.hub_check = (getenv("VSG_HUB_CHECK") && atoi(getenv("VSG_HUB_CHECK")) != 0) ? 1 : 0;
// ... 1101 lines not shown
          idx = next_region_index_++;
          key_to_region_.emplace(rep_key, idx);
          regions_.emplace_back();
          regions_.back().index = idx;
          regions_.back().size = sz[0];
          regions_.back().constrained_id = cons[0];
        } else {
          idx = it->second;
        }
        if (idx != r && idx > r && idx < num_regions) dirty[idx] = 1;
        regions_[idx].has_raster = true;
        regions_[idx].raster.swap(tr.tubes[k]);
      }
    }
  }

  for (const auto& kv : size_adjust) {
    auto it = key_to_region_.find(kv.first);
    if (it == key_to_region_.end()) {
      key_size_override_[kv.first] = 0;
      continue;
    }
    regions_[it->second].size += kv.second;
  }
  const double t_host1 = NowMs();

  const int n_rl = (int)rl_ty.size();
  if (n_rl > 0) {
    DevBuf<uint32_t>& d_ty = Grow(rl_ty_, n_rl);
    DevBuf<int32_t>&d_lx = Grow(rl_lx_, n_rl), &d_rx = Grow(rl_rx_, n_rl), &d_nl = Grow(rl_nl_, n_rl);
    H2D(d_ty.get(), rl_ty.data(), (size_t)n_rl, stream_);
    H2D(d_lx.get(), rl_lx.data(), (size_t)n_rl, stream_);
    H2D(d_rx.get(), rl_rx.data(), (size_t)n_rl, stream_);
    H2D(d_nl.get(), rl_new.data(), (size_t)n_rl, stream_);
    LaunchRelabelIntervals(d_ty.get(), d_lx.get(), d_rx.get(), d_nl.get(), n_rl, W_, H_,
                           label_uf_.get(), stream_);
    VSG_HIP(hipStreamSynchronize(stream_));
  }
  const int L = (int)lists_.size();
  int capacity = (int)std::max<size_t>(pairs_.size(), (size_t)1 << 20);
  int count = 0;
  bool hashed = false;
  if (!getenv("VSG_PAIR_TABLE") || atoi(getenv("VSG_PAIR_TABLE")) != 0) {
    const size_t cap = (size_t)1 << 21;
    pairs_sorted_.ensure(cap);
    pairs_unique_.ensure(cap);
    pairs_.ensure((size_t)capacity);
    order_keys_.ensure((size_t)capacity);
    PairTable table{pairs_sorted_.get(), pairs_unique_.get(), (unsigned)(cap - 1)};
    LaunchNeighborPairsHashed(list_desc_dev_.get(), L, label_uf_.get(), W_, table, scalars_.get() + 3, stream_);
    int distinct = 0;
    D2H(&distinct, scalars_.get() + 3, 1, stream_);
    VSG_HIP(hipStreamSynchronize(stream_));
    if (distinct <= (int)(cap / 2) && distinct <= capacity) {
      LaunchPairTableCompact(table, pairs_.get(), order_keys_.get(), scalars_.get() + 3, stream_);
      D2H(&count, scalars_.get() + 3, 1, stream_);
      VSG_HIP(hipStreamSynchronize(stream_));
      VSG_REQUIRE(count == distinct, -4, "pair table: entries lost");
      hashed = true;
    }
  }
  for (int attempt = 0; attempt < 2 && !hashed; ++attempt) {
    pairs_.ensure((size_t)capacity);
    order_keys_.ensure((size_t)capacity);
    LaunchNeighborPairs(list_desc_dev_.get(), L, label_uf_.get(), W_, pairs_.get(),
                        order_keys_.get(), scalars_.get() + 3, capacity, stream_);
    D2H(&count, scalars_.get() + 3, 1, stream_);
    VSG_HIP(hipStreamSynchronize(stream_));
    if (count <= capacity) break;
    VSG_REQUIRE(attempt == 0, -4, "neighbour pair buffer overflow");
    capacity = count + 1024;
  }
  std::vector<unsigned long long> uniq;
  if (count > 0) {
    pairs_sorted_.ensure((size_t)count);
    pairs_unique_.ensure((size_t)count);
    size_t temp = std::max(SortKeysU64TempBytes(count), UniqueU64TempBytes(count));
    if (temp > cub_temp_.size()) cub_temp_.alloc(temp);
    SortKeysU64(cub_temp_.get(), cub_temp_.size(), pairs_.get(), pairs_sorted_.get(), count, stream_);
    UniqueU64(cub_temp_.get(), cub_temp_.size(), pairs_sorted_.get(), pairs_unique_.get(),
              scalars_.get() + 4, count, stream_);
    int nu = 0;
    D2H(&nu, scalars_.get() + 4, 1, stream_);
    VSG_HIP(hipStreamSynchronize(stream_));
    uniq.resize(nu);
    D2H(uniq.data(), pairs_unique_.get(), (size_t)nu, stream_);
    VSG_HIP(hipStreamSynchronize(stream_));
  }
  const double t_dev2 = NowMs();

  std::vector<int32_t> unseen;
  for (unsigned long long pr : uniq) {
    const int ka = (int)(uint32_t)(pr >> 32), kb = (int)(uint32_t)(pr & 0xFFFFFFFFull);
    if (!key_to_region_.count(ka)) unseen.push_back(ka);
    if (!key_to_region_.count(kb)) unseen.push_back(kb);
  }
  std::sort(unseen.begin(), unseen.end());
  unseen.erase(std::unique(unseen.begin(), unseen.end()), unseen.end());
  if (!unseen.empty()) {
    const int U = (int)unseen.size();
    DevBuf<int32_t>& d_keys = Grow(un_keys_, U);
    DevBuf<unsigned long long>& d_min = Grow(un_min_, U);
    H2D(d_keys.get(), unseen.data(), (size_t)U, stream_);
    VSG_HIP(hipMemsetAsync(d_min.get(), 0xFF, (size_t)U * sizeof(unsigned long long), stream_));
    LaunchFirstOrderOfKeys(pairs_.get(), order_keys_.get(), count, d_keys.get(), U, d_min.get(),
                           stream_);
    std::vector<unsigned long long> h_min(U);
    D2H(h_min.data(), d_min.get(), (size_t)U, stream_);
    VSG_HIP(hipStreamSynchronize(stream_));
    std::vector<int> order(U);
    for (int i = 0; i < U; ++i) order[i] = i;
    std::sort(order.begin(), order.end(), [&](int a, int b) { return h_min[a] < h_min[b]; });
    std::vector<int32_t> sz, cons;
    fetch_states(unseen, &sz, &cons);
    for (int oi : order) {
      const int key = unseen[oi];
      const int idx = next_region_index_++;
      key_to_region_.emplace(key, idx);
      regions_.emplace_back();
      RegionInfo& ri = regions_.back();
      ri.index = idx;
      auto ov = key_size_override_.find(key);
      ri.size = (ov != key_size_override_.end()) ? ov->second : sz[oi];
      ri.constrained_id = cons[oi];
      ri.has_raster = false;
    }
  }
  for (unsigned long long pr : uniq) {
    const int ka = (int)(uint32_t)(pr >> 32), kb = (int)(uint32_t)(pr & 0xFFFFFFFFull);
    const int ia = key_to_region_.at(ka), ib = key_to_region_.at(kb);
    regions_[ia].neighbors.push_back(ib);
    regions_[ib].neighbors.push_back(ia);
  }
  for (RegionInfo& ri : regions_) {
    std::sort(ri.neighbors.begin(), ri.neighbors.end());
    ri.neighbors.erase(std::unique(ri.neighbors.begin(), ri.neighbors.end()), ri.neighbors.end());
  }
  const double t_end = NowMs();
  if (getenv("VSG_DEBUG_STATS")) {
    std::fprintf(stderr, "[vsg] readout: device1 %.1f host1 %.1f device2 %.1f host2 %.1f ms (intervals %d, pairs %d, unique %zu)\n",
                 t_dev1 - t_start, t_host1 - t_dev1, t_dev2 - t_host1, t_end - t_dev2, num_iv, count,
                 uniq.size());
    std::fprintf(stderr, "[vsg]   host1: region table %.1f, tube prepare %.1f, flow samples %.1f, tube finish %.1f, "
                 "bookkeeping %.1f ms (%zu regions, %lld matched tubes, at most %d in a region)\n", th[0] - t_dev1,
                 th[1] - th[0], th[2] - th[1], th[3] - th[2], t_host1 - th[3], regions_.size(), sum_tubes, most_tubes);
  }
  timings_.readout_ms = (float)((t_dev1 - t_start) + (t_dev2 - t_host1));
  timings_.host_post_ms = (float)((t_host1 - t_dev1) + (t_end - t_dev2));
}

void DenseGraphHip::CopySpatialBuckets(int t, uint16_t* out) {
  VSG_REQUIRE(t >= 0 && t < num_frames_ && lists_[2 * t].used, -1, "no spatial list for slice");
  ListBuf& lb = lists_[2 * t];
  std::vector<uint32_t> slots(lb.n);
  std::vector<int32_t> offs(kBucketSlots);
  D2H(slots.data(), lb.slots.get(), (size_t)lb.n, stream_);
  D2H(offs.data(), lb.offsets.get(), (size_t)kBucketSlots, stream_);
  VSG_HIP(hipStreamSynchronize(stream_));
  for (size_t i = 0; i < 4 * wh_; ++i) out[i] = 0xFFFF;
  for (int b = 0; b <= kNumBuckets; ++b) {
    for (int p = offs[b]; p < offs[b + 1]; ++p) {
      const uint32_t s = slots[p];
      out[(size_t)(s & 3u) * wh_ + (s >> 2)] = (uint16_t)b;
    }
  }
}

void DenseGraphHip::CopyTemporalBuckets(int t, uint16_t* out, int32_t* prev_idx) {
  VSG_REQUIRE(t >= 1 && t < num_frames_ && lists_[2 * t - 1].used, -1, "no temporal list");
  ListBuf& lb = lists_[2 * t - 1];
  std::vector<uint32_t> slots(lb.n);
  std::vector<int32_t> offs(kBucketSlots);
  D2H(slots.data(), lb.slots.get(), (size_t)lb.n, stream_);
  D2H(offs.data(), lb.offsets.get(), (size_t)kBucketSlots, stream_);
  D2H(prev_idx, lb.prev_idx.get(), wh_, stream_);
  VSG_HIP(hipStreamSynchronize(stream_));
  for (size_t i = 0; i < 9 * wh_; ++i) out[i] = 0xFFFF;
  for (int b = 0; b <= kNumBuckets; ++b) {
    for (int p = offs[b]; p < offs[b + 1]; ++p) {
      const uint32_t s = slots[p];
      const uint32_t pix = s / 9u, k = s - pix * 9u;
      out[(size_t)k * wh_ + pix] = (uint16_t)b;
    }
  }
}

void DenseGraphHip::CopyNodeRoots(int32_t* out) {
  const size_t N = wh_ * (size_t)num_frames_;
  LaunchFlatten(nodes(), N, label_uf_.get(), stream_);
  D2H(out, label_uf_.get(), N, stream_);
  VSG_HIP(hipStreamSynchronize(stream_));
}

void DenseGraphHip::CopyNodeStates(int32_t* root, float* mean, int32_t* size, int32_t* cons,
                                   uint8_t* flags) {
  const size_t N = wh_ * (size_t)num_frames_;
  if (N == 0) return;
  DevBuf<int32_t> d_root(N), d_cons(N), d_flags(N);
  DevBuf<float4> d_ds(N);
  std::vector<float4> h_ds(N);
  std::vector<int32_t> h_flags(N);
  LaunchFlatten(nodes(), N, d_root.get(), stream_);
  LaunchGatherStates(nodes(), d_root.get(), (int)N, d_ds.get(), d_cons.get(), d_flags.get(), stream_);
  D2H(root, d_root.get(), N, stream_);
  D2H(h_ds.data(), d_ds.get(), N, stream_);
  D2H(cons, d_cons.get(), N, stream_);
  D2H(h_flags.data(), d_flags.get(), N, stream_);
  VSG_HIP(hipStreamSynchronize(stream_));
  for (size_t i = 0; i < N; ++i) {
    mean[3 * i + 0] = h_ds[i].x;
    mean[3 * i + 1] = h_ds[i].y;
    mean[3 * i + 2] = h_ds[i].z;
    std::memcpy(&size[i], &h_ds[i].w, sizeof(int32_t));
    flags[i] = (uint8_t)h_flags[i];
  }
}

}
```

### video_segment_amd/csrc/dense_graph.h

```cpp
#ifndef VSG_DENSE_GRAPH_H_
#define VSG_DENSE_GRAPH_H_

#include <memory>
#include <unordered_map>
#include <vector>

#include "device_graph.h"
#include "host_model.h"

namespace vsg {

struct MergePaths {
  int64_t hub_stages = 0, hub_absorbed = 0;
  int64_t hub_cuts = 0, hub_cuts_in_groups = 0, hub_parts_in_later_bucket = 0, spine_side_cuts = 0;
  int64_t hub_retries = 0, hub_reasons[6] = {0, 0, 0, 0, 0, 0};
  int64_t hub_exclusion_reruns = 0, hub_off_reruns = 0, group_halvings = 0, conservative_replays = 0;
};

struct GraphTimings {
  float edges_ms = 0, sort_ms = 0, merge_ms = 0, readout_ms = 0, host_post_ms = 0;
  int64_t edges_total = 0, edges_active = 0;
  int64_t merges[3] = {0, 0, 0};
  float wave_ms = 0, filter_ms = 0, spine_ms = 0;
  int64_t wave_launches = 0, filter_launches = 0, wave_edges = 0, spine_launches = 0, spine_edges = 0;
  int64_t optimistic_stages = 0, rollbacks = 0;
  int64_t stages = 0;
  int64_t slab_growths = 0, spine_growths = 0;
  double slab_growth_ms = 0, spine_growth_ms = 0;
  int64_t runtime_mallocs = 0, runtime_frees = 0, cache_hits = 0, device_syncs = 0;
  double runtime_malloc_ms = 0, runtime_free_ms = 0, device_sync_ms = 0;
  int64_t mail_waits = 0;
  double mail_wait_ms = 0, mail_wait_longest_ms = 0;
  int mail_mode = 0;
  double segment_wall_ms = 0, prepare_ms = 0, constrained_merge_ms = 0;
  MergePaths paths;
  SpinePaths spine_paths = {};
};

class DenseGraphHip {
 public:
  DenseGraphHip(int W, int H, int max_frames, bool l1, hipStream_t stream);
  ~DenseGraphHip();

  int W() const { return W_; }
  int H() const { return H_; }
  int max_frames() const { return max_frames_; }
  int num_frames() const { return num_frames_; }
  hipStream_t stream() const { return stream_; }
  hipStream_t aux_stream() const { return aux_stream_; }

  void Reset(int max_frames);
  void ForgetLearned();

  void AddFrame(const float* feat_planar_dev, const int32_t* cons_dev);
  void AddVirtualFrame(const int32_t* ids_dev, int max_label);
  void AddVirtualFrameDeferred();
  void SetHaloLabels(const int32_t* virtual_ids_dev, const int32_t* constrained_ids_dev,
                     int max_label);
  bool halo_pending() const { return halo_pending_; }
  void AddTemporal(const float* cur_dev, const float* prev_dev, const float* flow_dev,
                   bool is_virtual);
  void FinishBuilding();
  void Segment(int min_region_size, bool force_constraints) {
    SegmentLists(min_region_size, force_constraints, spatial_pass_done_ ? 2 : 0);
  }
  void SegmentSpatially() {
    SegmentLists(0, false, 1);
    spatial_pass_done_ = true;
  }
  void ObtainResults(const std::vector<const float*>* dev_flows, bool enforce_n4,
                     bool enforce_spatial_connectedness);

  std::vector<RegionInfo>& regions() { return regions_; }
  const std::vector<RegionInfo>& regions() const { return regions_; }
  const GraphTimings& timings() const { return timings_; }

  void CopySpatialBuckets(int t, uint16_t* out_host);
  void CopyTemporalBuckets(int t, uint16_t* out_host, int32_t* prev_idx_host);
  void CopyNodeRoots(int32_t* out_host);
  void CopyNodeStates(int32_t* root, float* mean, int32_t* size, int32_t* cons, uint8_t* flags);

 private:
  struct ListBuf {
    DevBuf<uint32_t> slots;
    DevBuf<int32_t> offsets;
    DevBuf<int32_t> prev_idx;
    DevBuf<uint16_t> keys_dbg;
    int type = 0;
    int n = 0;
    int base_a = 0, base_b = 0;
    bool used = false;
  };

  void EnsureScratch(size_t n_edges_max);
  void EnsureActiveScratch(size_t n_active_max);
  void DebugHash(const char* where);
  void SortList(ListBuf& lb, int per_px);
  void MergeConstrainedHostAssisted();
  NodeArrays nodes() {
    return NodeArrays{parent_.get(), desc_sz_.get(), cons_.get(), flags_.get(), hub8_.get()};
  }

  QuiesceGuard quiesce_;
  int W_, H_, capacity_frames_, max_frames_;
  bool l1_;
  hipStream_t stream_;
  hipStream_t aux_stream_ = nullptr;
  hipStream_t aux2_stream_ = nullptr;
  hipEvent_t aux_fork_ = nullptr, aux_join_ = nullptr;
  int num_frames_ = 0;
  size_t wh_;
  bool has_constraints_ = false;
  std::vector<int> virtual_slices_;
  int min_region_size_ = 0;
  bool flattened_ = false;

  DevBuf<int32_t> parent_;
  DevBuf<float4> desc_sz_;
  DevBuf<int32_t> cons_;
  DevBuf<uint8_t> flags_;
  DevBuf<uint8_t> hub8_;
  DevBuf<int32_t> cc_, label_uf_, label_img_, adjust_;
  std::vector<ListBuf> lists_;
  DevBuf<ListDesc> list_desc_dev_;
  DevBuf<uint32_t> list_slot_base_dev_;
  std::vector<uint32_t> list_slot_base_;
  DevBuf<uint8_t> kept_all_;
  DevBuf<uint8_t> kept_spatial_pass_;
  bool spatial_pass_done_ = false;
  bool halo_pending_ = false;
  int deferred_virtual_slice_ = -1, deferred_constrained_slice_ = -1;
  void SegmentLists(int min_region_size, bool force_constraints, int pass);
  void RunStageDebug(int b, int w, int windows, int j0, int n, const MergeParams& P, int inert_mode,
                     MergeScratch& S, bool debug_stages, StageInfo* info);
  DevBuf<int32_t> bucket_base_dev_;
  std::vector<int32_t> bucket_base_host_;
  DevBuf<uint16_t> keys_tmp_;
  DevBuf<int32_t> hist_tmp_, hist_sums_;
  DevBuf<int32_t> first_label_scratch_;
  DevBuf<int32_t> e_ra_, e_rb_;
  DevBuf<uint32_t> e_gpos_;
  DevBuf<uint8_t> active_slab_;
  struct ActiveArrays {
    int32_t *e_active = nullptr, *e_apos = nullptr, *a_ra = nullptr, *a_rb = nullptr, *seg_cnt = nullptr,
            *seg_off = nullptr, *lead_pos = nullptr, *l_ra = nullptr, *l_rb = nullptr, *bk_cons = nullptr;
    uint32_t *a_gpos = nullptr, *a_comp = nullptr, *a_idx = nullptr, *s_comp = nullptr, *s_idx = nullptr,
             *seg_key = nullptr, *l_gpos = nullptr;
    float4* bk_ds = nullptr;
    uint8_t* bk_flags = nullptr;
  } act_;
  DevBuf<unsigned long long> filter_masks_;
  DevBuf<int32_t> block_cnt_, block_off_;
  int64_t optimistic_stages_ = 0, rollbacks_ = 0;
  DevBuf<int32_t> scalars_;
  DevBuf<int32_t> seg_table_dev_;
  DevBuf<int32_t> hub_excl_;
  PinnedBuf<int32_t> iv_host_;
  std::vector<int32_t> seg_table_host_, list_off_host_;
  size_t stage_ring_used_ = 0;
  PinnedBuf<int32_t> stage_ring_;
  Mailbox mail_;
  void* mail_mem_ = nullptr;
  DevBuf<int32_t> zero_pool_mem_;
  ZeroPool zero_pool_;
  DevBuf<int32_t> bucket_prefix_dev_;
  int spine_limit_bucket_ = 0x7fffffff;
  int spine_limit_age_ = 0;
  int spine_low_fails_[2] = {0, 0}, spine_low_cooldown_[2] = {0, 0};
  double spine_low_cost_fail_[2] = {0, 0}, spine_low_cost_skip_[2] = {0, 0};
  int spine_low_cost_age_[2] = {0, 0};
  DevBuf<int32_t> spine_pool_;
  static constexpr int64_t kNoWindowTarget = 1ll << 40;
  int64_t wave_target_active_ = kNoWindowTarget;
  std::vector<int64_t> window_target_;
  int window_target_age_ = 0;
  std::vector<int> window_last_seg_;
  std::vector<uint8_t> window_frozen_;
  std::vector<uint8_t> window_unpaid_;
  std::vector<int> window_peak_;
  std::vector<int> hub_bucket_stages_, hub_bucket_pause_;
  std::vector<long long> hub_bucket_absorbed_;
  double last_density_ = 1.0;
  int spine_max_edges_grown_ = 0;
  DevBuf<unsigned long long> stats_;
  DevBuf<uint8_t> cub_temp_;
  DevBuf<int32_t> scan_sums_;
  size_t scratch_edges_ = 0;
  size_t scratch_active_ = 0;
  DevBuf<int32_t> flow_req_dev_;
  DevBuf<float2> flow_samples_dev_;
  DevBuf<const float*> flow_ptrs_dev_;
  void SampleFlows(const std::vector<FlowRequest>& req, const std::vector<const float*>& dev_flows,
                   std::vector<float>* samples);
  DevBuf<int32_t> row_counts_, row_offsets_;
  DevBuf<int32_t> iv_label_, iv_lx_, iv_rx_;
  DevBuf<uint32_t> iv_ty_;
  DevBuf<unsigned long long> pairs_, order_keys_, pairs_sorted_, pairs_unique_;
  DevBuf<int32_t> small_i32_a_, small_i32_b_, small_i32_c_;
  DevBuf<float4> small_f4_;
  DevBuf<int32_t> mc_ids_, mc_par_, mc_cons_, mc_fl_, rl_lx_, rl_rx_, rl_nl_, un_keys_;
  DevBuf<float4> mc_ds_;
  DevBuf<uint32_t> rl_ty_;
  DevBuf<unsigned long long> un_min_;
  std::vector<hipEvent_t> ev_pool_;
  std::vector<std::pair<int, int>> ev_wave_, ev_filter_, ev_spine_;
  int ev_used_ = 0;

  std::vector<RegionInfo> regions_;
  std::unordered_map<int, int> key_to_region_;
  std::unordered_map<int, int> key_size_override_;
  int next_region_index_ = 0;
  GraphTimings timings_;
};

}

#endif
```

### video_segment_amd/csrc/device_graph.h

```cpp
#ifndef VSG_DEVICE_GRAPH_H_
#define VSG_DEVICE_GRAPH_H_

#include <functional>

#include "common.h"

namespace vsg {

constexpr uint8_t kFlagFinalized = 1;
constexpr uint8_t kFlagNoDesc = 2;
constexpr uint8_t kFlagTentative = 4;
constexpr uint8_t kFlagHub = 8;
constexpr uint8_t kFlagHubBroken = 16;
constexpr uint8_t kFlagHubExcluded = 32;
constexpr int kHubExclCap = 16384;
constexpr int kHubMaxAttempts = 4;
constexpr int kHubMaxSplits = 64;
constexpr int kHubCutCap = 64;
constexpr int kHubListInts = 4 + kHubExclCap + 3 * kHubCutCap;

struct NodeArrays {
  int32_t* parent;
  float4* desc_sz;
  int32_t* cons;
  uint8_t* flags;
  uint8_t* hub8;
};

struct ListDesc {
  const uint32_t* slots;
  uint8_t* kept;
  const int32_t* prev_idx;
  const int32_t* offsets;
  int32_t type;
  int32_t base_a;
  int32_t base_b;
  int32_t n;
};

struct MergeParams {
  int W, H;
  int num_lists;
  int min_region_size;
  float force_merge_weight;
  float inv_scale;
  float s_lt_005, s_lt_02, s_le_015;
  const uint8_t* spatial_survivors;
};

void UploadSpaceWeights(const float* w49, hipStream_t stream);
void LaunchMinMax(const uint8_t* bgr, size_t stride, int W, int H, int* mm, hipStream_t s);
void LaunchBilateral(const uint8_t* bgr, size_t stride, int W, int H, const float* lut,
                     float scale, float* planes, hipStream_t s);
void LaunchGaussian3(const uint8_t* bgr, size_t stride, int W, int H, float k0, float k1, float* planes,
                     hipStream_t s);
void LaunchConvertPlanar(const uint8_t* bgr, size_t stride, int W, int H, float* planes,
                         hipStream_t s);
void LaunchInterleavedToPlanar(const float* in, size_t n, float* planes, hipStream_t s);
void LaunchPlanarToInterleaved(const float* planes, size_t n, float* out, hipStream_t s);
size_t EdgeSortHistInts(size_t n_px);
size_t EdgeSortSumInts(size_t n_px);
void LaunchSpatialKeys(const float* feat, int W, int H, int l1, uint16_t* keys, int32_t* hist,
                       hipStream_t s);
void LaunchTemporalKeys(const float* cur, const float* prev, const float* flow, int W, int H,
                        int l1, int is_virtual, uint16_t* keys, int32_t* prev_idx, int32_t* hist,
                        hipStream_t s);
void LaunchBucketSort(const uint16_t* keys, size_t n_px, int per_px, int32_t* hist, int32_t* sums,
                      int32_t* offsets, uint32_t* slots_out, hipStream_t s);
void LaunchInitNodes(const float* feat, size_t n, int base, const int32_t* cons_in,
                     NodeArrays nodes, hipStream_t s);
void LaunchInitVirtualNodes(const int32_t* labels, size_t n, int base, int num_labels,
                            int32_t* first_scratch, NodeArrays nodes, hipStream_t s);

constexpr int kScanMaxTiles = 4096;
struct ScanScratch {
  int32_t* sums;
  hipStream_t owner = nullptr;
};

void DebugExclusiveSum(const ScanScratch& sc, const int32_t* in, int32_t* out, int n, int32_t* total, hipStream_t s);

size_t SortPairsU32HandTempBytes(int n);
void SortPairsU32Hand(void* temp, size_t temp_bytes, const uint32_t* keys_in, uint32_t* keys_out,
                      const uint32_t* vals_in, uint32_t* vals_out, int n, int end_bit, hipStream_t s);
size_t SortPairsU32LibTempBytes(int n);
void SortPairsU32Lib(void* temp, size_t temp_bytes, const uint32_t* keys_in, uint32_t* keys_out,
                     const uint32_t* vals_in, uint32_t* vals_out, int n, int end_bit, hipStream_t s);
size_t SortPairsU32TempBytes(int n);
void SortPairsU32(void* temp, size_t temp_bytes, const uint32_t* keys_in, uint32_t* keys_out,
                  const uint32_t* vals_in, uint32_t* vals_out, int n, int end_bit, hipStream_t s);
bool SortPairsU32TakesHand(int n);
size_t SortKeysU64TempBytes(int n);
void SortKeysU64(void* temp, size_t temp_bytes, const unsigned long long* in,
                 unsigned long long* out, int n,
                 hipStream_t s);
size_t UniqueU64TempBytes(int n);
void UniqueU64(void* temp, size_t temp_bytes, const unsigned long long* in,
               unsigned long long* out,
               int32_t* num_out, int n, hipStream_t s);

constexpr int kMailValues = 4;
struct MailSlot {
  unsigned long long* dev;
  volatile unsigned long long* host;
  unsigned seq;
};
struct Mailbox {
  unsigned long long* dev = nullptr;
  volatile unsigned long long* host = nullptr;
  int slots = 0;
  int next = 0;
  unsigned seq = 0;
  int32_t* list_dev = nullptr;
  volatile int32_t* list_host = nullptr;
  int list_cap = 0;
};
inline MailSlot NextMail(Mailbox& m) {
  MailSlot s{m.dev + (size_t)kMailValues * m.next, m.host + (size_t)kMailValues * m.next, ++m.seq};
  m.next = (m.next + 1) % m.slots;
  return s;
}
void MailWait(const MailSlot& slot, int count, int* values, hipStream_t s);
void MailRegisterGraph(int delta);
int MailYieldMode();
struct MailWaitCounters {
  long long waits = 0;
  double wait_ms = 0, longest_ms = 0;
};
MailWaitCounters MailWaitSnapshot();
void MailWaitResetLongest();
void LaunchMailPost(const MailSlot& slot, const int32_t* p0, const int32_t* p1, const int32_t* p2,
                    const int32_t* p3, hipStream_t s);

constexpr size_t kZeroArenaInts = 1024;
struct ZeroPool {
  int32_t* base = nullptr;
  size_t cap = 0, used = 0;
  bool second_half = false;
  size_t arena_used = 0;
};

struct FilterMasks {
  unsigned long long* active;
  unsigned long long* settled;
  unsigned long long* tentative;
  int32_t* block_cnt;
};
struct FilterSegRec {
  const uint32_t* slots;
  const int32_t* prev;
  int32_t start, pos0, type, base_a, base_b;
  uint32_t slot_base;
};
constexpr int kFilterArgSegs = 64;
struct FilterSegArgs {
  FilterSegRec r[kFilterArgSegs];
};
struct FilterSegs {
  const FilterSegRec* rec;
  int n;
};
constexpr size_t kStageRingInts = (size_t)1 << 18;
struct SpinePaths {
  int64_t replays, components, nested_replays, deepest_level;
  int64_t forest_rounds, forest_rounds_ahead, forest_compactions_ahead, forest_compactions_sync, forest_lists_refused;
  int64_t ranked_by_sampling, ranked_plain, rank_sampling_refused;
  int64_t jump_loops_ended_early, streamed_passes, streamed_refused;
  int64_t pool_fallbacks[4], top_level_fallbacks, nested_fallbacks;
  int64_t assumption_reruns, limit_bucket_moves, low_bucket_failures[2], low_bucket_skips[2];
  int64_t zero_pool_flips;
  int64_t windows_run, rle_stages, wide_launches, group_stages, sorts_hand, sorts_library;
};
struct MergeScratch {
  int active_cap;
  std::function<bool(long long need)> grow_active;
  int32_t* e_ra;
  int32_t* e_rb;
  uint32_t* e_gpos;
  int32_t* e_active;
  int32_t* e_apos;
  FilterMasks masks;
  int32_t* block_off;
  int32_t* a_ra;
  int32_t* a_rb;
  uint32_t* a_gpos;
  uint32_t* a_comp;
  uint32_t* a_idx;
  uint32_t* s_comp;
  uint32_t* s_idx;
  uint32_t* seg_key;
  int32_t* seg_cnt;
  int32_t* seg_off;
  int32_t* num_active;
  int32_t* num_segs;
  float4* bk_ds;
  int32_t* bk_cons;
  uint8_t* bk_flags;
  int force_rollback;
  int32_t* lead_pos;
  int32_t* l_ra;
  int32_t* l_rb;
  uint32_t* l_gpos;
  int use_rle;
  int group_hi;
  const int32_t* bucket_prefix;
  const int32_t* bucket_prefix_host;
  const int32_t* bucket_base_host;
  const int32_t* list_off_host;
  int32_t* seg_dev;
  size_t seg_cap;
  std::vector<int32_t>* seg_host;
  const ListDesc* lists_host;
  int filter_segs_mode;
  int32_t* ring_host;
  size_t ring_cap, *ring_used;
  int spine_min;
  int spine_off;
  int* spine_low_failed;
  const int* spine_low_skip;
  int* spine_limit_bucket;
  int spine_nested_factor;
  int spine_max_edges;
  int spine_debug, spine_check;
  int rank_split_min;
  int spine_fast;
  int spine_fast_min;
  int32_t* spine_pool;
  size_t spine_pool_ints;
  std::function<bool(long long edges)> grow_spine_pool;
  int32_t* nmap[3];
  hipStream_t aux_stream;
  hipStream_t aux2_stream;
  hipEvent_t aux_fork, aux_join;
  int small_seg;
  int wide_min;
  int wide_waves;
  int chain_relax;
  int hubs;
  int hubs_off;
  int hub_attempt;
  int hub_splits_left;
  int hub_split_depth;
  int hub_list_dirty;
  int hub_max_splits;
  int hub_cut_min_work;
  long long hub_splits;
  const uint32_t* list_slot_base_host;
  int32_t* hub_excl;
  long long hub_retries;
  long long hub_reasons[6];
  long long hub_cuts_in_groups;
  long long hub_parts_in_later_bucket;
  long long spine_side_cuts;
  long long hub_exclusion_reruns;
  long long hub_off_reruns;
  long long group_halvings;
  long long conservative_replays;
  long long hub_cut_ratio;
  int hub_check;
  SpinePaths sp;
  int wave_debug;
  int wave_dbg;
  int64_t* optimistic_stages;
  int64_t* rollbacks;
  int32_t* cc;
  unsigned long long* stats;
  void* cub_temp;
  size_t cub_temp_bytes;
  ScanScratch scan;
  int node_key_bits;
  std::vector<hipEvent_t>* ev_pool;
  std::vector<std::pair<int, int>>* ev_wave;
  std::vector<std::pair<int, int>>* ev_filter;
  std::vector<std::pair<int, int>>* ev_spine;
  int* ev_used;
  Mailbox* mail;
  ZeroPool* zeros;
  hipStream_t main_stream;
};
int32_t* TakeZeroed(MergeScratch& S, size_t n);

int32_t* TakeStageScalars(MergeScratch& S, size_t n);

int32_t* TakeStageRing(MergeScratch& S, size_t n);

void LaunchBuildBucketTable(const ListDesc* lists, int num_lists, int32_t* bucket_base,
                            hipStream_t s);
void LaunchInitIdentity(int32_t* a, size_t n, hipStream_t s);
struct StageInfo {
  int want_components = 0;
  int replayed = 0;
  int components = 0;
  int max_wave_segment = 0;
  int hub_stages = 0;
  long long hub_absorbed = 0;
  int hub_retries = 0;
};
void ResetHubExclusions(MergeScratch& S, NodeArrays nodes, hipStream_t s);
void RunBucketStage(int bucket, int j0, int n_b, const ListDesc* lists, const int32_t* bucket_base,
                    const uint32_t* list_slot_base, uint8_t* kept_all, NodeArrays nodes,
                    const MergeParams& P, int inert_mode, MergeScratch& S, hipStream_t s,
                    StageInfo* info = nullptr);
size_t SpinePoolInts(size_t max_edges);
void LaunchKeepVirtualBucket(const ListDesc* lists, int num_lists, hipStream_t s);

void LaunchFlatten(NodeArrays nodes, size_t n, int32_t* label_uf, hipStream_t s);
void LaunchEnforceN4(int32_t* label_img, int W, int H, const int32_t* frames_dev, int num_frames,
                     int32_t* row_flags , int32_t* adjust ,
                     hipStream_t s);
void LaunchRowRunCounts(const int32_t* label_img, int W, int H, const int32_t* frames_dev, int num_frames,
                        int32_t* row_counts , hipStream_t s);
struct IntervalArrays {
  int32_t* label;
  uint32_t* ty;
  int32_t* lx;
  int32_t* rx;
};
void LaunchWriteIntervals(const int32_t* label_img, int W, int H, const int32_t* frames_dev, int num_frames,
                          const int32_t* row_offsets ,
                          IntervalArrays out, hipStream_t s);
void LaunchRelabelIntervals(const uint32_t* ty, const int32_t* lx, const int32_t* rx,
                            const int32_t* new_label, int n, int W, int H, int32_t* label_uf,
                            hipStream_t s);
struct PairTable {
  unsigned long long* key;
// ... 36 lines not shown
```

### video_segment_amd/csrc/edge_sort.hip

```cpp
#include "merge_common.h"

namespace vsg {

constexpr int kTilePxSpatial = 2048;
constexpr int kTilePxTemporal = 1024;
constexpr int kBinInvalid = kBucketSlots - 1;

__device__ __forceinline__ float ColorDist(float ab, float ag, float ar, float bb, float bg,
                                           float br, int l1) {
  const float d1 = ab - bb, d2 = ag - bg, d3 = ar - br;
  if (l1) {
    return (float)((fabs((double)d1) + fabs((double)d2) + fabs((double)d3)) *
                   (double)(1.0f / 3.0f));
  }
  return sqrtf((d1 * d1 + d2 * d2 + d3 * d3) * (1.0f / 3.0f));
}

__device__ __forceinline__ uint16_t BucketOf(float w) {
  const float scale = 2048.0f / (1.0f + 1e-6f);
  return (uint16_t)(int)fminf(2048.0f, w * scale);
}

__device__ __forceinline__ int TruncToIntX86(float v) {
  if (!(v < 2147483648.0f && v >= -2147483648.0f)) return (int)0x80000000;
// ... 107 lines not shown
        }
      }
    }
    __syncthreads();
    const int px_here = (int)min((size_t)256, n - pix0);
    const int words = (px_here * 9 + 1) / 2;
    uint32_t* out32 = reinterpret_cast<uint32_t*>(keys + pix0 * 9);
    const uint32_t* in32 = reinterpret_cast<const uint32_t*>(stage);
    if ((px_here * 9) & 1) {
      for (int w = threadIdx.x; w < words - 1; w += 256) out32[w] = in32[w];
      if (threadIdx.x == 0) keys[pix0 * 9 + (size_t)px_here * 9 - 1] = stage[px_here * 9 - 1];
    } else {
      for (int w = threadIdx.x; w < words; w += 256) out32[w] = in32[w];
    }
    __syncthreads();
  }
  StoreTileHist(lds_hist, blockIdx.x, num_tiles, hist);
}

constexpr int kScanPerBlock = 2048;

__device__ __forceinline__ int BlockExclusiveScan256(int v, int32_t* lds4, int& total) {
  const int lane = threadIdx.x & 63, wave = threadIdx.x >> 6;
  const int incl = WaveInclusiveSum(v);
  if (lane == 63) lds4[wave] = incl;
  __syncthreads();
  int before = 0;
  for (int w = 0; w < wave; ++w) before += lds4[w];
  total = lds4[0] + lds4[1] + lds4[2] + lds4[3];
  __syncthreads();
  return before + incl - v;
}

__global__ __launch_bounds__(256) void k_scan_block_sums(const int32_t* __restrict__ a, int n,
                                                          int32_t* __restrict__ sums) {
  __shared__ int32_t lds4[4];
  const int base = blockIdx.x * kScanPerBlock + threadIdx.x * 8;
  int v = 0;
#pragma unroll
  for (int k = 0; k < 8; ++k) v += (base + k < n) ? a[base + k] : 0;
  int total;
  BlockExclusiveScan256(v, lds4, total);
  if (threadIdx.x == 0) sums[blockIdx.x] = total;
}

__global__ __launch_bounds__(256) void k_scan_sums(int32_t* __restrict__ sums, int m) {
  __shared__ int32_t lds4[4];
  int carry = 0;
  for (int base = 0; base < m; base += 256) {
    const int i = base + threadIdx.x;
    const int v = i < m ? sums[i] : 0;
    int total;
    const int ex = BlockExclusiveScan256(v, lds4, total);
    if (i < m) sums[i] = carry + ex;
    carry += total;
  }
}

__global__ __launch_bounds__(256) void k_scan_apply(int32_t* __restrict__ a, int n,
                                                     const int32_t* __restrict__ sums,
                                                     int num_tiles, int32_t* __restrict__ offsets) {
  __shared__ int32_t lds4[4];
  const int base = blockIdx.x * kScanPerBlock + threadIdx.x * 8;
  int x[8];
  int v = 0;
#pragma unroll
  for (int k = 0; k < 8; ++k) {
    x[k] = (base + k < n) ? a[base + k] : 0;
    v += x[k];
  }
  int total;
  int run = sums[blockIdx.x] + BlockExclusiveScan256(v, lds4, total);
#pragma unroll
  for (int k = 0; k < 8; ++k) {
    const int i = base + k;
    if (i < n) {
      a[i] = run;
      if (i % num_tiles == 0) offsets[i / num_tiles] = run;
    }
    run += x[k];
  }
}

__device__ __forceinline__ unsigned long long SameBinMask(int bin) {
  unsigned long long m = ~0ull;
#pragma unroll
  for (int b = 0; b < 12; ++b) {
    const unsigned long long bal = __ballot((bin >> b) & 1);
    m &= ((bin >> b) & 1) ? bal : ~bal;
  }
  return m;
}

template <int kPerPx, int kTilePx>
__global__ __launch_bounds__(256) void k_scatter_slots(const uint16_t* __restrict__ keys,
                                                        size_t n_px,
                                                        const int32_t* __restrict__ scanned,
                                                        int num_tiles,
                                                        uint32_t* __restrict__ slots_out) {
  constexpr int kTileSlots = kTilePx * kPerPx;
  __shared__ __attribute__((aligned(16))) uint16_t lds_keys[kTileSlots];
  __shared__ int32_t cnt[4][kBucketSlots];
  const int tile = blockIdx.x;
  const size_t px0 = (size_t)tile * kTilePx;
  const int n_slots = (int)(min((size_t)kTilePx, n_px - px0) * kPerPx);
  const int lane = threadIdx.x & 63, wave = threadIdx.x >> 6;
  for (int b = threadIdx.x; b < 4 * kBucketSlots; b += 256) (&cnt[0][0])[b] = 0;
  {
    const uint32_t* in32 = reinterpret_cast<const uint32_t*>(keys + px0 * kPerPx);
    uint32_t* l32 = reinterpret_cast<uint32_t*>(lds_keys);
    const int words = n_slots >> 1;
    for (int w = threadIdx.x; w < words; w += 256) l32[w] = in32[w];
    if ((n_slots & 1) && threadIdx.x == 0) lds_keys[n_slots - 1] = keys[px0 * kPerPx + n_slots - 1];
  }
  __syncthreads();
  const int quarter = ((n_slots + 255) / 256) * 64;
  const int q_beg = min(n_slots, wave * quarter), q_end = min(n_slots, (wave + 1) * quarter);
  for (int i = q_beg + lane; i < q_end; i += 64) {
    const int key = lds_keys[i];
    atomicAdd(&cnt[wave][key == kInvalidKey ? kBinInvalid : key], 1);
  }
  __syncthreads();
  for (int b = threadIdx.x; b < kBucketSlots; b += 256) {
    const int c0 = cnt[0][b], c1 = cnt[1][b], c2 = cnt[2][b], c3 = cnt[3][b];
    if ((c0 | c1 | c2 | c3) == 0) continue;
    const int run = scanned[(size_t)b * num_tiles + tile];
    cnt[0][b] = run;
    cnt[1][b] = run + c0;
    cnt[2][b] = run + c0 + c1;
    cnt[3][b] = run + c0 + c1 + c2;
  }
  __syncthreads();
  const uint32_t slot0 = (uint32_t)(px0 * kPerPx);
  for (int i0 = q_beg; i0 < q_end; i0 += 64) {
    const int i = i0 + lane;
    const bool valid = i < q_end;
    const int key = valid ? (int)lds_keys[i] : (int)kInvalidKey;
    const int bin = key == kInvalidKey ? kBinInvalid : key;
    const unsigned long long same = SameBinMask(bin);
    const int rank = (int)__popcll(same & ((1ull << lane) - 1ull));
    const int start = cnt[wave][bin];
    if (valid && bin != kBinInvalid) slots_out[start + rank] = slot0 + (uint32_t)i;
    __builtin_amdgcn_wave_barrier();
    if (rank == 0) cnt[wave][bin] = start + (int)__popcll(same);
    __builtin_amdgcn_fence(__ATOMIC_SEQ_CST, "wavefront");
    __builtin_amdgcn_wave_barrier();
  }
}

static int NumTiles(size_t n_px, int per_px) {
  const int tile = per_px == 4 ? kTilePxSpatial : kTilePxTemporal;
  return (int)((n_px + tile - 1) / tile);
}
size_t EdgeSortHistInts(size_t n_px) { return (size_t)kBucketSlots * NumTiles(n_px, 9); }
size_t EdgeSortSumInts(size_t n_px) {
  return (EdgeSortHistInts(n_px) + kScanPerBlock - 1) / kScanPerBlock;
}

void LaunchSpatialKeys(const float* feat, int W, int H, int l1, uint16_t* keys, int32_t* hist,
                       hipStream_t s) {
  const int T = NumTiles((size_t)W * H, 4);
  VSG_HIP(hipMemsetAsync(hist, 0, (size_t)kBucketSlots * T * sizeof(int32_t), s));
  hipLaunchKernelGGL(k_spatial_keys, dim3(T), dim3(256), 0, s, feat, W, H, l1,
                     reinterpret_cast<ushort4*>(keys), hist, T);
  VSG_HIP(hipGetLastError());
}

void LaunchTemporalKeys(const float* cur, const float* prev, const float* flow, int W, int H,
                        int l1, int is_virtual, uint16_t* keys, int32_t* prev_idx, int32_t* hist,
                        hipStream_t s) {
  const int T = NumTiles((size_t)W * H, 9);
  VSG_HIP(hipMemsetAsync(hist, 0, (size_t)kBucketSlots * T * sizeof(int32_t), s));
  hipLaunchKernelGGL(k_temporal_keys, dim3(T), dim3(256), 0, s, cur, prev, flow, W, H, l1,
                     is_virtual, keys, prev_idx, hist, T);
  VSG_HIP(hipGetLastError());
}

void LaunchBucketSort(const uint16_t* keys, size_t n_px, int per_px, int32_t* hist, int32_t* sums,
                      int32_t* offsets, uint32_t* slots_out, hipStream_t s) {
  const int T = NumTiles(n_px, per_px);
  const int n = kBucketSlots * T;
  const int blocks = (n + kScanPerBlock - 1) / kScanPerBlock;
  hipLaunchKernelGGL(k_scan_block_sums, dim3(blocks), dim3(256), 0, s, hist, n, sums);
  hipLaunchKernelGGL(k_scan_sums, dim3(1), dim3(256), 0, s, sums, blocks);
  hipLaunchKernelGGL(k_scan_apply, dim3(blocks), dim3(256), 0, s, hist, n, sums, T, offsets);
  if (per_px == 4) {
    hipLaunchKernelGGL((k_scatter_slots<4, kTilePxSpatial>), dim3(T), dim3(256), 0, s, keys, n_px,
                       hist, T, slots_out);
  } else {
    hipLaunchKernelGGL((k_scatter_slots<9, kTilePxTemporal>), dim3(T), dim3(256), 0, s, keys, n_px,
                       hist, T, slots_out);
  }
  VSG_HIP(hipGetLastError());
}

}
```

### video_segment_amd/csrc/stream.cpp

```cpp
#include "stream.h"

#include <atomic>
#include <exception>
#include <thread>

#include <algorithm>
#include <chrono>
#include <cmath>
#include <cstdio>
#include <cstring>

namespace vsg {

namespace {
double NowMs() {
  using clk = std::chrono::steady_clock;
  return std::chrono::duration<double, std::milli>(clk::now().time_since_epoch()).count();
}
}

Preprocessor::Preprocessor(int W, int H, hipStream_t stream) : W_(W), H_(H), stream_(stream) {
  minmax_dev_.alloc(2);
}

const Preprocessor::Lut& Preprocessor::GetLut(int umin, int umax) {
  auto key = std::make_pair(umin, umax);
  auto it = luts_.find(key);
  if (it != luts_.end()) return *it->second;
  const float c255 = (float)(1.0 / 255.0);
  const double min_val = (double)((float)umin * c255);
  const double max_val = (double)((float)umax * c255);
  const int cn = 3;
  const float sigma_color = 0.25f;
  const float diff_range = std::max<float>(
      1e-3f, (float)((max_val - min_val) * (max_val - min_val) * cn * (double)1.02f));
  const int num_bins = (1 << 12) * cn;
  const float scale = (float)num_bins / diff_range;
  const float color_coeff = (float)(-0.5 / (double)(sigma_color * sigma_color));
  std::vector<float> lut(num_bins);
  bool zero_reached = false;
  for (int i = 0; i < num_bins; ++i) {
    if (!zero_reached) {
      lut[i] = (float)std::exp((double)((float)i / scale * color_coeff));
      zero_reached = ((double)lut[i] < 1e-10);
    } else {
      lut[i] = 0;
    }
  }
  std::unique_ptr<Lut> l(new Lut);
  l->table.alloc((size_t)num_bins);
  l->scale = scale;
  VSG_HIP(hipMemcpyAsync(l->table.get(), lut.data(), lut.size() * sizeof(float),
                         hipMemcpyHostToDevice, stream_));
  VSG_HIP(hipStreamSynchronize(stream_));
  if (luts_.size() > 64) luts_.clear();
  auto res = luts_.emplace(key, std::move(l));
  return *res.first->second;
}

void Preprocessor::Run(const uint8_t* bgr_dev, size_t stride, int presmoothing, float* out) {
  const double t0 = NowMs();
  if (presmoothing == 0) {
    LaunchConvertPlanar(bgr_dev, stride, W_, H_, out, stream_);
  } else if (presmoothing == 1) {
    float cf[3];
    double sum = 0;
    const double scale2x = -0.5 / (1.5 * 1.5);
    for (int i = 0; i < 3; ++i) {
      const double x = i - 1.0;
      cf[i] = (float)std::exp(scale2x * x * x);
      sum += cf[i];
    }
    sum = 1.0 / sum;
    for (int i = 0; i < 3; ++i) cf[i] = (float)(cf[i] * sum);
    LaunchGaussian3(bgr_dev, stride, W_, H_, cf[1], cf[0], out, stream_);
  } else {
    VSG_REQUIRE(presmoothing == 2, -1, "presmoothing has to be 0 (none), 1 (gaussian) or 2 (bilateral)");
    if (!space_uploaded_) {
      float w[49];
      const float sigma_space = 3.0f;
      const int radius = (int)(sigma_space * 1.5f);
      const float coeff = -0.5f / (sigma_space * sigma_space);
      int k = 0;
      for (int i = -radius; i <= radius; ++i) {
        for (int j = -radius; j <= radius; ++j) {
          const int r2 = i * i + j * j;
          if (r2 > radius * radius) continue;
          w[k++] = (float)std::exp((double)(coeff * (float)r2));
        }
      }
      VSG_REQUIRE(k == 49, -4, "unexpected bilateral window");
      UploadSpaceWeights(w, stream_);
      space_uploaded_ = true;
    }
    LaunchMinMax(bgr_dev, stride, W_, H_, minmax_dev_.get(), stream_);
    int mm[2] = {0, 0};
    VSG_HIP(hipMemcpyAsync(mm, minmax_dev_.get(), sizeof(mm), hipMemcpyDeviceToHost, stream_));
    VSG_HIP(hipStreamSynchronize(stream_));
    const Lut& lut = GetLut(mm[0], mm[1]);
    LaunchBilateral(bgr_dev, stride, W_, H_, lut.table.get(), lut.scale, out, stream_);
  }
  last_ms_ = (float)(NowMs() - t0);
}

DenseSegmentationHip::DenseSegmentationHip(const vsg_options& o, int W, int H)
    : options_(o), W_(W), H_(H), wh_((size_t)W * H) {
  VSG_REQUIRE(options_.chunk_size >= 3, -1, "Chunk size needs to be at least 3 frames.");
  overlap_frames_ = (int)(options_.chunk_overlap_ratio * (float)options_.chunk_size + 0.5f);
  overlap_frames_ = std::min(overlap_frames_, 2);
  VSG_REQUIRE(overlap_frames_ < options_.chunk_size, -1, "Overlap needs to be smaller than chunk_size.");
  VSG_REQUIRE(overlap_frames_ == 2, -1, "chunk_overlap_ratio too small: the reference needs a 2 frame overlap");
  VSG_REQUIRE(options_.num_constraint_frames >= 1, -1, "num_constraint_frames >= 1");
  constraint_frames_ = std::min(options_.num_constraint_frames, overlap_frames_ - 1);
  VSG_HIP(hipStreamCreateWithFlags(&stream_, hipStreamNonBlocking));
  graph_.reset(new DenseGraphHip(W, H, options_.chunk_size + 1, options_.color_distance == 0, stream_));
  input_stream_ = graph_->aux_stream();
  VSG_HIP(hipEventCreateWithFlags(&input_done_, hipEventDisableTiming));
  pre_.reset(new Preprocessor(W, H, input_stream_));
  planes_ = std::make_shared<PlanePool>();
  std::memset(&last_timings_, 0, sizeof(last_timings_));
  std::memset(&accum_, 0, sizeof(accum_));
}

DenseSegmentationHip::~DenseSegmentationHip() {
  quiesce_.Begin();
  if (stream_) {
    (void)hipStreamSynchronize(stream_);
    if (input_done_) (void)hipEventDestroy(input_done_);
    for (hipEvent_t e : edge_ev_) (void)hipEventDestroy(e);
    graph_.reset();
    pre_.reset();
    feature_buffer_.clear();
    flow_dev_buffer_.clear();
    planes_.reset();
    (void)hipStreamDestroy(stream_);
  }
  if (halo_ids_host_) CacheFree(halo_ids_host_);
}

int DenseSegmentationHip::MinRegionSize() const {
  return (int)(options_.frac_min_region_size * (float)W_ * options_.frac_min_region_size *
               (float)H_ * (float)options_.chunk_size);
}

int DenseSegmentationHip::ProcessFrame(bool flush, const uint8_t* bgr, size_t stride,
                                       const float* flow, bool has_flow_stream, int mem) {
  results_.clear();
  encoded_.clear();
  if (forget_pending_) {
    graph_->ForgetLearned();
    forget_pending_ = false;
  }
  if (!graph_open_) {
    graph_->Reset(options_.chunk_size);
    graph_open_ = true;
    seg_chunk_id_ = chunk_id_;
  }
  if (bgr) {
    VSG_REQUIRE(stride >= (size_t)W_ * 3, -1, "stride smaller than a row");
    struct InputDrain {
      hipStream_t s;
      bool armed = true;
      ~InputDrain() {
        if (armed) (void)hipStreamSynchronize(s);
      }
    } drain{input_stream_};
    const uint8_t* bgr_dev = bgr;
    if (mem == VSG_MEM_HOST) {
      staging_bgr_.ensure(stride * (size_t)H_);
      VSG_HIP(hipMemcpyAsync(staging_bgr_.get(), bgr, stride * (size_t)(H_ - 1) + (size_t)W_ * 3,
                             hipMemcpyHostToDevice, input_stream_));
      bgr_dev = staging_bgr_.get();
    }
    DevPlane feat = planes_->Take(3 * wh_);
    pre_->Run(bgr_dev, stride, options_.presmoothing, feat->get());
    accum_.preprocess_ms += pre_->last_ms();
    accum_.preprocess_launches += 1;

    VSG_REQUIRE(frames_fed_ == 0 || has_flow_stream == flow_stream_seen_, -1,
                "has_flow_stream changed in the middle of a stream");
    ++frames_fed_;
    if (has_flow_stream) {
      flow_stream_seen_ = true;
      if (frames_fed_ == 1 && !pending_import_) {
        flow_dev_buffer_.push_back(nullptr);
      } else {
        VSG_REQUIRE(flow != nullptr, -1, "Flow always has to be passed or be absent.");
        DevPlane fd = planes_->Take(2 * wh_);
        VSG_HIP(hipMemcpyAsync(fd->get(), flow, 2 * wh_ * sizeof(float),
                               mem == VSG_MEM_HOST ? hipMemcpyHostToDevice : hipMemcpyDeviceToDevice,
                               input_stream_));
        flow_dev_buffer_.push_back(fd);
      }
    }
    VSG_HIP(hipEventRecord(input_done_, input_stream_));
    VSG_HIP(hipStreamWaitEvent(stream_, input_done_, 0));

    const bool first_after_import = pending_import_;
    const int ev = TakeEdgeEvents();
    try {
    VSG_HIP(hipEventRecord(edge_ev_[(size_t)ev], stream_));
    if (pending_import_) {
      feature_buffer_.push_back(nullptr);
      feature_buffer_.push_back(feat);
      if (has_flow_stream) {
        DevPlane fd = flow_dev_buffer_.back();
        flow_dev_buffer_.clear();
        flow_dev_buffer_.push_back(nullptr);
        flow_dev_buffer_.push_back(fd);
      }
      curr_chunk_start_ = 1;
      if (halo_deferred_) {
        StartConstrainedGraph(nullptr, nullptr, 0);
      } else {
        StartConstrainedGraph(halo_ids_dev_[0].get(), halo_ids_dev_[1].get(), pending_max_label_);
      }
      pending_import_ = false;
    } else {
      feature_buffer_.push_back(feat);
      graph_->AddFrame(feat->get(), nullptr);
      if (feature_buffer_.size() > 1) {
        const float* fl = flow_dev_buffer_.empty() ? nullptr : flow_dev_buffer_.back()->get();
        graph_->AddTemporal(feature_buffer_.end()[-1]->get(), feature_buffer_.end()[-2]->get(), fl,
                            false);
      }
    }
    VSG_HIP(hipEventRecord(edge_ev_[(size_t)ev + 1], stream_));
    } catch (...) {
      edge_ev_used_ = ev;
      throw;
    }
    if (first_after_import) {
      VSG_HIP(hipStreamSynchronize(stream_));
    }
    VSG_HIP(hipEventSynchronize(input_done_));
    drain.armed = false;
    accum_.edge_launches += 1;
    ++input_frames_;
  }
  if (flush || (int)feature_buffer_.size() - curr_chunk_start_ >= options_.chunk_size) {
    ChunkBoundaryOutput(flush);
    return (int)results_.size();
  }
  return 0;
}

int DenseSegmentationHip::TakeEdgeEvents() {
  while ((size_t)edge_ev_used_ + 2 > edge_ev_.size()) {
    hipEvent_t e = nullptr;
    VSG_HIP(hipEventCreate(&e));
    edge_ev_.push_back(e);
  }
  edge_ev_used_ += 2;
  return edge_ev_used_ - 2;
}

void DenseSegmentationHip::StartConstrainedGraph(const int32_t* virt_ids_dev,
                                                 const int32_t* cons_ids_dev, int max_label) {
  graph_->Reset(curr_chunk_start_ + options_.chunk_size);
  graph_open_ = true;
  seg_chunk_id_ = chunk_id_;
  if (virt_ids_dev) {
    graph_->AddVirtualFrame(virt_ids_dev, std::max(max_label, 1));
  } else {
    graph_->AddVirtualFrameDeferred();
  }
  graph_->AddFrame(feature_buffer_[1]->get(), cons_ids_dev);
  const float* fl = flow_dev_buffer_.empty() ? nullptr : flow_dev_buffer_[1]->get();
  graph_->AddTemporal(nullptr, nullptr, fl, true);
}

void DenseSegmentationHip::ChunkBoundaryOutput(bool flush) {
  const double tb0 = NowMs();
  SegmentAndOutputChunk(flush);
  const double tb1 = NowMs();
  if (flush) {
    graph_open_ = false;
    return;
  }
  VSG_REQUIRE((int)overlap_segmentations_.size() == constraint_frames_ + 1, -4, "overlap size");
  const double tb2 = NowMs();
  StartConstrainedGraph(halo_ids_dev_[0].get(), halo_ids_dev_[1].get(), max_region_id_);
  overlap_segmentations_.clear();
  if (getenv("VSG_DEBUG_STATS")) {
    VSG_HIP(hipStreamSynchronize(stream_));
    std::fprintf(stderr, "[vsg] boundary: segment+output %.1f ms, halo planes %.1f ms (%d in the pool), next graph start %.1f ms\n",
                 tb1 - tb0, tb2 - tb1, (int)boundary_paths_.halo_planes_in_pool, NowMs() - tb2);
  }
}

void DenseSegmentationHip::SegmentAndOutputChunk(bool flush) {
  std::vector<const float*> flows;
  const bool have_flows = !flow_dev_buffer_.empty();
  if (have_flows) {
    for (const auto& f : flow_dev_buffer_) flows.push_back(f ? f->get() : nullptr);
  }
  graph_->FinishBuilding();
  for (int k = 0; k + 1 < edge_ev_used_; k += 2) {
    float ms = 0;
    VSG_HIP(hipEventElapsedTime(&ms, edge_ev_[(size_t)k], edge_ev_[(size_t)k + 1]));
    accum_.edges_ms += ms;
  }
  edge_ev_used_ = 0;
  if (options_.two_stage_oversegment) graph_->SegmentSpatially();
  graph_->Segment(MinRegionSize(), true);
  if (keep_node_states_) {
    const size_t n = wh_ * (size_t)graph_->num_frames();
    node_states_.root.resize(n);
    node_states_.size.resize(n);
    node_states_.constraint.resize(n);
    node_states_.mean.resize(3 * n);
    node_states_.flags.resize(n);
    graph_->CopyNodeStates(node_states_.root.data(), node_states_.mean.data(), node_states_.size.data(),
                           node_states_.constraint.data(), node_states_.flags.data());
  }
  graph_->ObtainResults(have_flows ? &flows : nullptr, options_.enforce_n4_connectivity != 0,
                        options_.enforce_spatial_connectedness != 0);
  const double t_host0 = NowMs();
  double t_h[6] = {0};
  const GraphTimings& gt = graph_->timings();
  last_merge_stats_[0] = gt.merges[0];
  last_merge_stats_[1] = gt.merges[1];
  last_merge_stats_[2] = gt.merges[2];

  const int buffered = (int)feature_buffer_.size();
  const int overlap_start = buffered - (flush ? 0 : overlap_frames_);
  const int last_output_frame = std::min(buffered - 1, overlap_start);
  VSG_REQUIRE(overlap_start > curr_chunk_start_, -3, "flush without buffered frames");
  const int max_result_frame = std::min(buffered - 1, last_output_frame + constraint_frames_);

  std::vector<RegionInfo>& regions = graph_->regions();
  const int lhs = 0, rhs = last_output_frame + 1;
  for (RegionInfo& r : regions) {
    if (!r.has_raster || r.raster.empty() || r.raster.front().frame >= rhs ||
        r.raster.back().frame < lhs) {
      r.removed = true;
    }
  }
  for (RegionInfo& r : regions) {
    if (!r.has_raster) continue;
    int inc = 0;
    for (const RasterSlice& sl : r.raster) {
      if (sl.frame < lhs || sl.frame >= rhs) inc -= RasterArea(sl.raster);
    }
    r.size += inc;
  }
  const bool use_constraints = chunk_id_ > 0;
  assigned_constrained_ids_ = use_constraints;
  int max_id = -1;
  for (RegionInfo& r : regions) {
    r.region_id = (use_constraints && r.constrained_id >= 0) ? r.constrained_id
                                                             : r.index + max_region_id_;
    max_id = std::max(max_id, r.region_id);
  }
  max_region_id_ = std::max(max_region_id_, max_id + 1);

  t_h[0] = NowMs();
  const int chunk_size = last_output_frame - curr_chunk_start_ + 1;
  overlap_segmentations_.clear();
  const int hierarchy_frame_idx = num_output_frames_;
  const int num_result_frames = max_result_frame - curr_chunk_start_ + 1;
  std::vector<std::unique_ptr<SegDesc>> descs((size_t)num_result_frames);
  std::vector<std::string> wires((size_t)num_result_frames);
  const int first_overlap_task = last_output_frame - curr_chunk_start_;
  const int num_halo_tasks = flush ? 0 : num_result_frames - first_overlap_task;
  if (!flush) {
    VSG_REQUIRE(num_halo_tasks == constraint_frames_ + 1 && num_halo_tasks == 2, -4, "overlap size");
    if (!halo_ids_host_) {
      halo_ids_host_ = static_cast<int32_t*>(CacheAlloc(2 * wh_ * sizeof(int32_t), kCachePinned));
    }
  }
  std::atomic<int> halo_planes(0);
  {
    std::atomic<int> next(0);
    std::mutex error_mu;
    std::exception_ptr error;
    auto work = [&]() {
      try {
        for (int j = next.fetch_add(1); j < num_result_frames; j = next.fetch_add(1)) {
          const int halo = (j >= 1 && j <= num_halo_tasks) ? j - 1 : -1;
          const int i = j == 0 ? 0 : halo >= 0 ? first_overlap_task + halo : j - num_halo_tasks;
          const int frame_idx = curr_chunk_start_ + i;
          std::unique_ptr<SegDesc> desc(new SegDesc());
          Retrieve(frame_idx, frame_idx == curr_chunk_start_, desc.get());
          desc->chunk_size = chunk_size;
          desc->overlap_start = chunk_size;
          desc->hierarchy_frame_idx = hierarchy_frame_idx;
          if (halo >= 0) {
            int32_t* ids = halo_ids_host_ + (size_t)halo * wh_;
            std::fill(ids, ids + wh_, -1);
            RenderIdImage(*desc, W_, ids);
            halo_planes.fetch_add(1);
          }
          if (frame_idx <= last_output_frame) wires[(size_t)i] = EncodeSegDesc(*desc);
          descs[(size_t)i] = std::move(desc);
        }
      } catch (...) {
        std::lock_guard<std::mutex> lock(error_mu);
        if (!error) error = std::current_exception();
        next.store(num_result_frames);
      }
    };
    const int hw = (int)std::thread::hardware_concurrency();
    const int num_threads = std::max(1, std::min({num_result_frames, hw > 0 ? hw : 1, 32}));
    std::vector<std::thread> pool;
    try {
      for (int t = 1; t < num_threads; ++t) pool.emplace_back(work);
    } catch (...) {
    }
    work();
    for (std::thread& t : pool) t.join();
    if (error) std::rethrow_exception(error);
  }
  boundary_paths_.halo_planes_in_pool = halo_planes.load();
  if (!flush) {
    for (int k = 0; k < 2; ++k) {
      halo_ids_dev_[k].ensure(wh_);
      VSG_HIP(hipMemcpyAsync(halo_ids_dev_[k].get(), halo_ids_host_ + (size_t)k * wh_, wh_ * sizeof(int32_t),
                             hipMemcpyHostToDevice, stream_));
    }
    halo_valid_ = true;
  }
  t_h[1] = NowMs();
  for (int i = 0; i < num_result_frames; ++i) {
    const int frame_idx = curr_chunk_start_ + i;
    std::unique_ptr<SegDesc>& desc = descs[(size_t)i];
    if (frame_idx < last_output_frame) {
      results_.push_back(std::move(desc));
      encoded_.push_back(std::move(wires[(size_t)i]));
      ++num_output_frames_;
      continue;
    }
    if (frame_idx == last_output_frame) {
      results_.push_back(std::unique_ptr<SegDesc>(new SegDesc(*desc)));
      encoded_.push_back(std::move(wires[(size_t)i]));
      ++num_output_frames_;
    }
    overlap_segmentations_.push_back(std::move(desc));
  }

  t_h[2] = NowMs();
  feature_buffer_.erase(feature_buffer_.begin(), feature_buffer_.begin() + last_output_frame);
  if (!flow_dev_buffer_.empty()) {
    flow_dev_buffer_.erase(flow_dev_buffer_.begin(), flow_dev_buffer_.begin() + last_output_frame);
  }
  curr_chunk_start_ = flush ? 0 : 1;
  if (!flush) {
    VSG_REQUIRE(overlap_frames_ == (int)feature_buffer_.size(), -4, "overlap buffer size");
    feature_buffer_[0].reset();
    if (!flow_dev_buffer_.empty()) {
// ... 173 lines not shown
```

### video_segment_amd/csrc/stream.h

```cpp
#ifndef VSG_STREAM_H_
#define VSG_STREAM_H_

#include <map>
#include <memory>
#include <mutex>
#include <string>
#include <vector>

#include "../../include/vsg.h"
#include "dense_graph.h"

namespace vsg {

class Preprocessor {
 public:
  Preprocessor(int W, int H, hipStream_t stream);
  void Run(const uint8_t* bgr_dev, size_t stride, int presmoothing, float* out_planar_dev);
  float last_ms() const { return last_ms_; }

 private:
  struct Lut {
    DevBuf<float> table;
    float scale = 0;
  };
  const Lut& GetLut(int umin, int umax);
  int W_, H_;
  hipStream_t stream_;
  DevBuf<int> minmax_dev_;
  std::map<std::pair<int, int>, std::unique_ptr<Lut>> luts_;
  bool space_uploaded_ = false;
  float last_ms_ = 0;
};

class PlanePool : public std::enable_shared_from_this<PlanePool> {
 public:
  typedef std::shared_ptr<DevBuf<float>> Plane;
  Plane Take(size_t n) {
    DevBuf<float>* b = nullptr;
    {
      std::lock_guard<std::mutex> lock(mu_);
      auto it = free_.find(n);
      if (it != free_.end()) {
        b = it->second;
        free_.erase(it);
      }
    }
    if (!b) b = new DevBuf<float>(n);
    std::weak_ptr<PlanePool> self = shared_from_this();
    return Plane(b, [self](DevBuf<float>* p) {
      if (auto pool = self.lock()) {
        std::lock_guard<std::mutex> lock(pool->mu_);
        pool->free_.emplace(p->size(), p);
      } else {
        delete p;
      }
    });
  }
  ~PlanePool() {
    for (auto& kv : free_) delete kv.second;
  }

 private:
  std::mutex mu_;
  std::multimap<size_t, DevBuf<float>*> free_;
};

class DenseSegmentationHip {
 public:
  DenseSegmentationHip(const vsg_options& o, int W, int H);
  ~DenseSegmentationHip();

  int ProcessFrame(bool flush, const uint8_t* bgr, size_t stride, const float* flow,
                   bool has_flow_stream, int mem);
  int ChunkSize() const { return options_.chunk_size; }

  int num_results() const { return (int)results_.size(); }
  const std::string& result_bytes(int i);
  const SegDesc& result(int i) const { return *results_[i]; }
  void last_merge_stats(int64_t* s3) const;
  struct NodeStates {
    std::vector<int32_t> root, size, constraint;
    std::vector<float> mean;
    std::vector<uint8_t> flags;
  };
  void keep_node_states(bool on) { keep_node_states_ = on; }
  const NodeStates& last_node_states() const { return node_states_; }
  const vsg_timings& last_timings() const { return last_timings_; }
  const GraphTimings& last_graph_timings() const { return last_graph_timings_; }
  const vsg_boundary_paths& last_boundary_paths() const { return boundary_paths_; }
  void CopyLastSmoothed(float* out_interleaved_host);
  int W() const { return W_; }
  int H() const { return H_; }

  void ExpectHalo();
  void Restart();
  void ExportHalo(const int32_t** virt, const int32_t** cons, int64_t scalars[4]);
  void ImportHalo(const int32_t* virt, const int32_t* cons, int mem, const int64_t scalars[4]);

 private:
  typedef std::shared_ptr<DevBuf<float>> DevPlane;
  int MinRegionSize() const;
  void ChunkBoundaryOutput(bool flush);
  void SegmentAndOutputChunk(bool flush);
  void StartConstrainedGraph(const int32_t* virt_ids_dev, const int32_t* cons_ids_dev,
                             int max_label);
  void Retrieve(int frame, bool output_hierarchy, SegDesc* desc) const;
  int TakeEdgeEvents();

  QuiesceGuard quiesce_;
  vsg_options options_;
  int W_, H_;
  size_t wh_;
  hipStream_t stream_ = nullptr;
  std::unique_ptr<DenseGraphHip> graph_;
  hipStream_t input_stream_ = nullptr;
  hipEvent_t input_done_ = nullptr;
  std::vector<hipEvent_t> edge_ev_;
  int edge_ev_used_ = 0;
  std::unique_ptr<Preprocessor> pre_;
  std::shared_ptr<PlanePool> planes_;
  bool graph_open_ = false;

  int input_frames_ = 0;
  int chunk_id_ = 0;
  int seg_chunk_id_ = 0;
  int overlap_frames_ = 2;
  int constraint_frames_ = 1;
  int max_region_id_ = 0;
  int num_output_frames_ = 0;
  int curr_chunk_start_ = 0;
  bool assigned_constrained_ids_ = false;

  std::vector<DevPlane> feature_buffer_;
  std::vector<DevPlane> flow_dev_buffer_;
  bool forget_pending_ = false;
  bool halo_deferred_ = false;
  bool flow_stream_seen_ = false;
  int64_t frames_fed_ = 0;

  DevBuf<uint8_t> staging_bgr_;
  DevBuf<float> staging_flow_;
  DevBuf<int32_t> halo_ids_dev_[2];
  int32_t* halo_ids_host_ = nullptr;
  bool halo_valid_ = false;
  bool pending_import_ = false;
  int pending_max_label_ = 0;

  std::vector<std::unique_ptr<SegDesc>> overlap_segmentations_;
  std::vector<std::unique_ptr<SegDesc>> results_;
  std::vector<std::string> encoded_;
  int64_t last_merge_stats_[3] = {0, 0, 0};
  bool keep_node_states_ = false;
  NodeStates node_states_;
  vsg_timings last_timings_;
  GraphTimings last_graph_timings_;
  vsg_boundary_paths boundary_paths_ = {0};
  vsg_timings accum_;
};

}

#endif
```

### video_segment_amd/dense_segmentation.py

```python
import ctypes as C

import numpy as np

from . import _lib
from ._lib import (VsgBoundaryPaths, VsgDiagnostics, VsgMergePaths, VsgOptions, VsgSpinePaths, VsgTimings, check,
                   lib)


def default_options(**kw):
    o = VsgOptions()
    lib().vsg_default_options(C.byref(o))
    for k, v in kw.items():
        setattr(o, k, v)
    return o


def _is_torch(x):
    return type(x).__module__.startswith("torch")


_DTYPE_NAMES = {"uint8": ("uint8",), "float32": ("float32",), "int32": ("int32",)}


def _ptr_mem(x, dtype=None, strided_rows=False):
    if x is None:
        return None, _lib.VSG_MEM_HOST
    name = str(x.dtype).replace("torch.", "")
    if dtype is not None and name != dtype:
        raise TypeError("expected %s, got %s" % (dtype, name))
    if _is_torch(x):
        if not (x.is_contiguous() or (strided_rows and x.dim() == 3 and x.stride(2) == 1
                                       and x.stride(1) == x.shape[2])):
            raise ValueError("tensor has to be contiguous")
        mem = _lib.VSG_MEM_DEVICE if x.is_cuda else _lib.VSG_MEM_HOST
        return C.c_void_p(x.data_ptr()), mem
    if not (x.flags["C_CONTIGUOUS"] or (strided_rows and x.ndim == 3 and x.strides[2] == x.itemsize
                                         and x.strides[1] == x.shape[2] * x.itemsize)):
        raise ValueError("array has to be C-contiguous")
    return x.ctypes.data_as(C.c_void_p), _lib.VSG_MEM_HOST


def _same_mem(mem_a, mem_b, what):
    if mem_a != mem_b:
        raise ValueError("%s has to live in the same memory kind (host / device) as the frame" % what)


def _row_stride(bgr):
    if _is_torch(bgr):
        assert bgr.stride(2) == 1 and bgr.stride(1) == 3
        return bgr.stride(0) * bgr.element_size()
    assert bgr.strides[2] == 1 and bgr.strides[1] == 3
    return bgr.strides[0]


class DenseSegmentation:

    def __init__(self, width, height, options=None, has_flow=False):
        self.W, self.H = width, height
        self.has_flow = has_flow
        self.opts = options if options is not None else default_options()
        h = C.c_void_p()
        check(lib().vsg_stream_create(C.byref(self.opts), width, height, C.byref(h)))
        self.h = h
        self._destroy = lib().vsg_stream_destroy

    def close(self):
        if getattr(self, "h", None):
            self._destroy(self.h)
            self.h = None

    def __del__(self):
        self.close()

    def chunk_size(self):
        return lib().vsg_stream_chunk_size(self.h)

    def process_frame(self, bgr, flow=None, flush=False):
        stride = 0
        if bgr is not None:
            assert tuple(bgr.shape) == (self.H, self.W, 3)
            stride = _row_stride(bgr)
        p_bgr, mem = _ptr_mem(bgr, "uint8", strided_rows=True)
        if flow is not None:
            assert tuple(flow.shape) == (self.H, self.W, 2)
            if not _is_torch(flow):
                flow = np.ascontiguousarray(flow, dtype=np.float32)
            p_flow, mem_f = _ptr_mem(flow, "float32")
            if bgr is not None:
                _same_mem(mem_f, mem, "the flow field")
            else:
                mem = mem_f
        else:
            p_flow = None
        n = C.c_int()
        check(lib().vsg_stream_process_frame(self.h, int(flush), p_bgr, stride, p_flow,
                                             int(self.has_flow), mem, C.byref(n)))
        self._n = n.value
        return n.value

    def result_bytes(self, i):
        p = C.c_void_p()
        n = C.c_size_t()
        check(lib().vsg_stream_result_bytes(self.h, i, C.byref(p), C.byref(n)))
        return C.string_at(p, n.value)

    def result_id_image(self, i):
        out = np.empty((self.H, self.W), np.int32)
        check(lib().vsg_stream_result_id_image(self.h, i, out.ctypes.data_as(C.c_void_p)))
        return out

    def last_merge_stats(self):
        s = np.zeros(3, np.int64)
        check(lib().vsg_stream_last_merge_stats(self.h, s.ctypes.data_as(C.c_void_p)))
        return s

    def keep_node_states(self, on=True):
        check(lib().vsg_stream_keep_node_states(self.h, int(on)))

    def last_node_states(self):
        n = C.c_int64()
        p = [C.c_void_p() for _ in range(5)]
        check(lib().vsg_stream_last_node_states(self.h, C.byref(n), *[C.byref(x) for x in p]))
        n = n.value

        def arr(ptr, ctype, count):
            return np.ctypeslib.as_array(C.cast(ptr, C.POINTER(ctype)), shape=(count,)).copy()
        return (arr(p[0], C.c_int32, n), arr(p[1], C.c_float, 3 * n).reshape(n, 3), arr(p[2], C.c_int32, n),
                arr(p[3], C.c_int32, n), arr(p[4], C.c_uint8, n))

    def last_timings(self):
        t = VsgTimings()
        check(lib().vsg_stream_last_timings(self.h, C.byref(t)))
        return t

    def last_diagnostics(self):
        d = VsgDiagnostics()
        check(lib().vsg_stream_last_diagnostics(self.h, C.byref(d)))
        return d.as_dict()

    def last_merge_paths(self):
        m = VsgMergePaths()
        check(lib().vsg_stream_last_merge_paths(self.h, C.byref(m)))
        return m.as_dict()

    def last_boundary_paths(self):
        m = VsgBoundaryPaths()
        check(lib().vsg_stream_last_boundary_paths(self.h, C.byref(m)))
        return m.as_dict()

    def last_spine_paths(self):
        m = VsgSpinePaths()
        check(lib().vsg_stream_last_spine_paths(self.h, C.byref(m)))
        return m.as_dict()

    def last_smoothed(self):
        out = np.empty((self.H, self.W, 3), np.float32)
        check(lib().vsg_stream_last_smoothed(self.h, out.ctypes.data_as(C.c_void_p)))
        return out

    def export_halo(self):
        a, b = C.c_void_p(), C.c_void_p()
        s = np.zeros(4, np.int64)
        check(lib().vsg_stream_export_halo(self.h, C.byref(a), C.byref(b),
                                           s.ctypes.data_as(C.c_void_p)))
        return a.value, b.value, s

    def expect_halo(self):
        check(lib().vsg_stream_expect_halo(self.h))

    def restart(self):
        check(lib().vsg_stream_restart(self.h))

    def import_halo(self, labels_virtual, labels_constrained, scalars):
        n = self.W * self.H
        for a in (labels_virtual, labels_constrained):
            if int(np.prod(tuple(a.shape))) != n:
                raise ValueError("label planes have to hold W*H int32")
        pa, mem = _ptr_mem(labels_virtual, "int32")
        pb, mem_b = _ptr_mem(labels_constrained, "int32")
        _same_mem(mem_b, mem, "the second label plane")
        s = np.ascontiguousarray(scalars, dtype=np.int64)
        check(lib().vsg_stream_import_halo(self.h, pa, pb, mem, s.ctypes.data_as(C.c_void_p)))


class ChunkChain:

    def __init__(self, rank, world, id_file, nonce=0, device=-1):
        h = C.c_void_p()
        check(lib().vsg_chain_create(rank, world, id_file.encode(), C.c_uint64(nonce), device,
                                     C.byref(h)))
        self.h = h
        self._destroy = lib().vsg_chain_destroy

    def close(self):
        if getattr(self, "h", None):
            self._destroy(self.h)
            self.h = None

    def __del__(self):
        self.close()

    def info(self):
        r, w = C.c_int(), C.c_int()
        check(lib().vsg_chain_info(self.h, C.byref(r), C.byref(w)))
        return r.value, w.value

    def send_halo(self, stream, dst):
        check(lib().vsg_chain_send_halo(self.h, stream.h, dst))

    def recv_halo(self, stream, src):
        check(lib().vsg_chain_recv_halo(self.h, stream.h, src))

    def exchange_halo(self, from_stream, dst, into_stream, src):
        check(lib().vsg_chain_exchange_halo(self.h, from_stream.h if from_stream else None, dst,
                                            into_stream.h if into_stream else None, src))


class DenseSegGraph:

    def __init__(self, width, height, max_frames, l1=False, device=-1):
        self.W, self.H, self.max_frames = width, height, max_frames
        h = C.c_void_p()
        check(lib().vsg_graph_create(width, height, max_frames, int(l1), device, C.byref(h)))
        self.h = h
        self._destroy = lib().vsg_graph_destroy

    def close(self):
        if getattr(self, "h", None):
            self._destroy(self.h)
            self.h = None

    def __del__(self):
        self.close()

    def add_frame_bgr(self, bgr, presmoothing=2, constraint_ids=None):
        assert tuple(bgr.shape) == (self.H, self.W, 3)
        p, mem = _ptr_mem(bgr, "uint8", strided_rows=True)
        if constraint_ids is not None and not _is_torch(constraint_ids):
            constraint_ids = np.ascontiguousarray(constraint_ids, np.int32)
        pc, mem_c = _ptr_mem(constraint_ids, "int32")
        if constraint_ids is not None:
            _same_mem(mem_c, mem, "constraint_ids")
        check(lib().vsg_graph_add_frame_bgr(self.h, p, _row_stride(bgr), presmoothing, pc, mem))

    def add_frame_features(self, feat, constraint_ids=None):
        if not _is_torch(feat):
            feat = np.ascontiguousarray(feat, np.float32)
        assert tuple(feat.shape) == (self.H, self.W, 3)
        p, mem = _ptr_mem(feat, "float32")
        if constraint_ids is not None and not _is_torch(constraint_ids):
            constraint_ids = np.ascontiguousarray(constraint_ids, np.int32)
        pc, mem_c = _ptr_mem(constraint_ids, "int32")
        if constraint_ids is not None:
            _same_mem(mem_c, mem, "constraint_ids")
        check(lib().vsg_graph_add_frame_features(self.h, p, pc, mem))

    def add_virtual_frame(self, constraint_ids):
        if not _is_torch(constraint_ids):
            constraint_ids = np.ascontiguousarray(constraint_ids, np.int32)
        p, mem = _ptr_mem(constraint_ids, "int32")
        check(lib().vsg_graph_add_virtual_frame(self.h, p, mem))

    def add_temporal(self, flow=None, is_virtual=False):
        if flow is not None and not _is_torch(flow):
            flow = np.ascontiguousarray(flow, np.float32)
        p, mem = _ptr_mem(flow, "float32")
        check(lib().vsg_graph_add_temporal(self.h, p, int(is_virtual), mem))

    def finish_building(self):
        check(lib().vsg_graph_finish_building(self.h))

    def segment_spatially(self):
        check(lib().vsg_graph_segment_spatially(self.h))

    def segment(self, min_region_size, force_constraints):
        check(lib().vsg_graph_segment(self.h, int(min_region_size), int(force_constraints)))

    def obtain_results(self, use_flows=False, enforce_n4=True, enforce_spatial_connectedness=True):
        check(lib().vsg_graph_obtain_results(self.h, int(use_flows), int(enforce_n4),
                                             int(enforce_spatial_connectedness)))

    def num_frames(self):
        return lib().vsg_graph_num_frames(self.h)

    def num_regions(self):
        return lib().vsg_graph_num_regions(self.h)

    def num_neighbor_links(self):
        return lib().vsg_graph_num_neighbor_links(self.h)

    def region_sizes(self):
        n = self.num_regions()
        s = np.empty(n, np.int32)
        c = np.empty(n, np.int32)
        check(lib().vsg_graph_region_sizes(self.h, s.ctypes.data_as(C.c_void_p),
                                           c.ctypes.data_as(C.c_void_p)))
        return s, c

    def index_image(self, t):
        out = np.empty((self.H, self.W), np.int32)
        check(lib().vsg_graph_index_image(self.h, t, out.ctypes.data_as(C.c_void_p)))
        return out
# ... 76 lines not shown
```

Measured before the change: 212.5.

## Build spatial edge lists on a side stream with separate sort scratch

```diff
diff --git a/include/vsg.h b/include/vsg.h
--- a/include/vsg.h
+++ b/include/vsg.h
@@ -130,6 +130,10 @@
   int64_t halo_planes_in_pool;
 } vsg_boundary_paths;
 
+typedef struct vsg_build_paths {
+  int64_t lists_on_side_stream;
+} vsg_build_paths;
+
 typedef struct vsg_memory_stats {
   int64_t bytes_in_use;
   int64_t bytes_in_use_peak;
@@ -166,6 +170,7 @@
 int vsg_stream_last_merge_paths(const vsg_stream* s, vsg_merge_paths* out);
 int vsg_stream_last_spine_paths(const vsg_stream* s, vsg_spine_paths* out);
 int vsg_stream_last_boundary_paths(const vsg_stream* s, vsg_boundary_paths* out);
+int vsg_stream_last_build_paths(const vsg_stream* s, vsg_build_paths* out);
 int vsg_stream_last_smoothed(vsg_stream* s, float* out);
 
 int vsg_stream_export_halo(vsg_stream* s, const int32_t** dev_labels_virtual,
diff --git a/video_segment_amd/_lib.py b/video_segment_amd/_lib.py
--- a/video_segment_amd/_lib.py
+++ b/video_segment_amd/_lib.py
@@ -96,8 +96,7 @@
         ("low_bucket_failures", C.c_int64 * 2), ("low_bucket_skips", C.c_int64 * 2),
         ("zero_pool_flips", C.c_int64),
         ("windows_run", C.c_int64), ("rle_stages", C.c_int64), ("wide_launches", C.c_int64),
-        ("group_stages", C.c_int64), ("sorts_hand", C.c_int64), ("sorts_library", C.c_int64),
-    ]
+        ("group_stages", C.c_int64), ("sorts_hand", C.c_int64), ("sorts_library", C.c_int64),    ]
 
     def as_dict(self):
         return {k: (list(getattr(self, k)) if issubclass(t, C.Array) else getattr(self, k)) for k, t in self._fields_}
@@ -106,6 +105,15 @@
 class VsgBoundaryPaths(C.Structure):
     _fields_ = [
         ("halo_planes_in_pool", C.c_int64),
+    ]
+
+    def as_dict(self):
+        return {k: getattr(self, k) for k, _ in self._fields_}
+
+
+class VsgBuildPaths(C.Structure):
+    _fields_ = [
+        ("lists_on_side_stream", C.c_int64),
     ]
 
     def as_dict(self):
@@ -144,7 +152,7 @@
     "vsg_stream_result_bytes", "vsg_stream_result_id_image", "vsg_stream_last_merge_stats",
     "vsg_stream_keep_node_states", "vsg_stream_last_node_states",
     "vsg_stream_last_timings", "vsg_stream_last_diagnostics", "vsg_stream_last_merge_paths", "vsg_stream_last_spine_paths",
-    "vsg_stream_last_boundary_paths",
+    "vsg_stream_last_boundary_paths", "vsg_stream_last_build_paths",
     "vsg_stream_last_smoothed", "vsg_stream_export_halo",
     "vsg_stream_import_halo", "vsg_stream_expect_halo", "vsg_stream_restart",
     "vsg_chain_create", "vsg_chain_destroy", "vsg_chain_info", "vsg_chain_send_halo",
@@ -210,6 +218,7 @@
     L.vsg_stream_last_merge_paths.argtypes = [vp, C.POINTER(VsgMergePaths)]
     L.vsg_stream_last_spine_paths.argtypes = [vp, C.POINTER(VsgSpinePaths)]
     L.vsg_stream_last_boundary_paths.argtypes = [vp, C.POINTER(VsgBoundaryPaths)]
+    L.vsg_stream_last_build_paths.argtypes = [vp, C.POINTER(VsgBuildPaths)]
     L.vsg_stream_last_smoothed.argtypes = [vp, vp]
     L.vsg_stream_export_halo.argtypes = [vp, C.POINTER(vp), C.POINTER(vp), vp]
     L.vsg_stream_import_halo.argtypes = [vp, vp, vp, C.c_int, vp]
diff --git a/video_segment_amd/csrc/capi.cpp b/video_segment_amd/csrc/capi.cpp
--- a/video_segment_amd/csrc/capi.cpp
+++ b/video_segment_amd/csrc/capi.cpp
@@ -411,6 +411,13 @@
   return Guard([&] {
     VSG_REQUIRE(s && out, VSG_ERR_INVALID, "null argument");
     *out = s->impl->last_boundary_paths();
+  });
+}
+
+int vsg_stream_last_build_paths(const vsg_stream* s, vsg_build_paths* out) {
+  return Guard([&] {
+    VSG_REQUIRE(s && out, VSG_ERR_INVALID, "null argument");
+    *out = s->impl->last_build_paths();
   });
 }
 
@@ -873,6 +880,7 @@
     g->timings.preprocess_launches += 1;
     const int32_t* ids = StageIds(g, constraint_ids, mem);
     g->g->AddFrame(feat->get(), ids);
+    g->g->JoinBuild();
     VSG_HIP(hipStreamSynchronize(g->stream));
     g->feats.push_back(feat);
     g->flows_dev.push_back(nullptr);
@@ -895,6 +903,7 @@
     vsg::LaunchInterleavedToPlanar(src, g->wh, feat->get(), g->stream);
     const int32_t* ids = StageIds(g, constraint_ids, mem);
     g->g->AddFrame(feat->get(), ids);
+    g->g->JoinBuild();
     VSG_HIP(hipStreamSynchronize(g->stream));
     g->feats.push_back(feat);
     g->flows_dev.push_back(nullptr);
diff --git a/video_segment_amd/csrc/dense_graph.cpp b/video_segment_amd/csrc/dense_graph.cpp
--- a/video_segment_amd/csrc/dense_graph.cpp
+++ b/video_segment_amd/csrc/dense_graph.cpp
@@ -59,6 +59,12 @@
   keys_tmp_.alloc(9 * wh_ + 8);
   hist_tmp_.alloc(EdgeSortHistInts(wh_));
   hist_sums_.alloc(EdgeSortSumInts(wh_) + 1);
+  if (const char* e = getenv("VSG_BUILD_STREAMS")) build_streams_ = atoi(e) == 1 ? 1 : 2;
+  if (build_streams_ == 2) {
+    keys_side_.alloc(4 * wh_ + 8);
+    hist_side_.alloc(EdgeSortHistInts(wh_, 4));
+    sums_side_.alloc(EdgeSortSumInts(wh_, 4) + 1);
+  }
   scalars_.alloc(32);
   stats_.alloc(96);
   hub_excl_.alloc(kHubListInts);
@@ -90,6 +96,8 @@
   VSG_HIP(hipStreamCreateWithFlags(&aux2_stream_, hipStreamNonBlocking));
   VSG_HIP(hipEventCreateWithFlags(&aux_fork_, hipEventDisableTiming));
   VSG_HIP(hipEventCreateWithFlags(&aux_join_, hipEventDisableTiming));
+  VSG_HIP(hipEventCreateWithFlags(&build_fork_, hipEventDisableTiming));
+  VSG_HIP(hipEventCreateWithFlags(&build_join_, hipEventDisableTiming));
 
   scan_sums_.alloc(kScanMaxTiles);
   Reset(max_frames);
@@ -97,11 +105,14 @@
 }
 
 DenseGraphHip::~DenseGraphHip() {
+  if (side_pending_ && aux2_stream_) (void)hipStreamSynchronize(aux2_stream_);
   quiesce_.Begin();
   MailRegisterGraph(-1);
   for (hipEvent_t e : ev_pool_) (void)hipEventDestroy(e);
   if (aux_fork_) (void)hipEventDestroy(aux_fork_);
   if (aux_join_) (void)hipEventDestroy(aux_join_);
+  if (build_fork_) (void)hipEventDestroy(build_fork_);
+  if (build_join_) (void)hipEventDestroy(build_join_);
   if (aux_stream_) (void)hipStreamDestroy(aux_stream_);
   if (aux2_stream_) (void)hipStreamDestroy(aux2_stream_);
   if (mail_mem_) CacheFree(mail_mem_);
@@ -109,6 +120,9 @@
 
 void DenseGraphHip::Reset(int max_frames) {
   VSG_REQUIRE(max_frames >= 1 && max_frames <= capacity_frames_, -1, "max_frames above capacity");
+  JoinBuild();
+  lists_on_side_ = 0;
+  side_forked_ = false;
   max_frames_ = max_frames;
   num_frames_ = 0;
   has_constraints_ = false;
@@ -139,27 +153,46 @@
   last_density_ = 1.0;
 }
 
-void DenseGraphHip::SortList(ListBuf& lb, int per_px) {
+void DenseGraphHip::SortList(ListBuf& lb, int per_px, const BuildScratch& bs) {
   const int n = (int)(per_px * wh_);
   lb.slots.ensure((size_t)n);
   lb.offsets.ensure(kBucketSlots);
-  LaunchBucketSort(keys_tmp_.get(), wh_, per_px, hist_tmp_.get(), hist_sums_.get(),
-                   lb.offsets.get(), lb.slots.get(), stream_);
+  LaunchBucketSort(bs.keys, wh_, per_px, bs.hist, bs.sums, lb.offsets.get(), lb.slots.get(), bs.stream);
   lb.n = n;
   lb.used = true;
 }
 
-void DenseGraphHip::AddFrame(const float* feat, const int32_t* cons_dev) {
+void DenseGraphHip::JoinBuild() {
+  if (!side_pending_) return;
+  VSG_HIP(hipEventRecord(build_join_, aux2_stream_));
+  VSG_HIP(hipStreamWaitEvent(stream_, build_join_, 0));
+  side_pending_ = false;
+}
+
+void DenseGraphHip::AddFrame(const float* feat, const int32_t* cons_dev, hipEvent_t planes_ready) {
   VSG_REQUIRE(num_frames_ < max_frames_, -1, "more frames than max_frames (CHECK_LE)");
   const int t = num_frames_;
   const int base = (int)(wh_ * t);
-  LaunchInitNodes(feat, wh_, base, cons_dev, nodes(), stream_);
+  BuildScratch bs = {keys_tmp_.get(), hist_tmp_.get(), hist_sums_.get(), stream_};
+  if (build_streams_ == 2) {
+    bs = BuildScratch{keys_side_.get(), hist_side_.get(), sums_side_.get(), aux2_stream_};
+    if (planes_ready && side_forked_) {
+      VSG_HIP(hipStreamWaitEvent(aux2_stream_, planes_ready, 0));
+    } else {
+      VSG_HIP(hipEventRecord(build_fork_, stream_));
+      VSG_HIP(hipStreamWaitEvent(aux2_stream_, build_fork_, 0));
+      side_forked_ = true;
+    }
+    side_pending_ = true;
+    ++lists_on_side_;
+  }
+  LaunchInitNodes(feat, wh_, base, cons_dev, nodes(), bs.stream);
   ListBuf& lb = lists_[2 * t];
   lb.type = 0;
   lb.base_a = base;
   lb.base_b = base;
-  LaunchSpatialKeys(feat, W_, H_, l1_ ? 1 : 0, keys_tmp_.get(), hist_tmp_.get(), stream_);
-  SortList(lb, 4);
+  LaunchSpatialKeys(feat, W_, H_, l1_ ? 1 : 0, bs.keys, bs.hist, bs.stream);
+  SortList(lb, 4, bs);
   if (cons_dev) has_constraints_ = true;
   ++num_frames_;
 }
@@ -192,6 +225,7 @@
   VSG_REQUIRE(num_frames_ > deferred_constrained_slice_, -3,
               "the constrained slice has to be added before its labels");
   VSG_REQUIRE(max_label >= 1, -1, "max_label must be positive");
+  JoinBuild();
   first_label_scratch_.ensure((size_t)max_label);
   LaunchInitVirtualNodes(virtual_ids_dev, wh_, (int)(wh_ * deferred_virtual_slice_), max_label,
                          first_label_scratch_.get(), nodes(), stream_);
@@ -211,10 +245,13 @@
   lb.prev_idx.ensure(wh_);
   LaunchTemporalKeys(cur, prev, flow, W_, H_, l1_ ? 1 : 0, is_virtual ? 1 : 0, keys_tmp_.get(),
                      lb.prev_idx.get(), hist_tmp_.get(), stream_);
-  SortList(lb, 9);
-}
-
-void DenseGraphHip::FinishBuilding() { VSG_HIP(hipStreamSynchronize(stream_)); }
+  SortList(lb, 9, BuildScratch{keys_tmp_.get(), hist_tmp_.get(), hist_sums_.get(), stream_});
+}
+
+void DenseGraphHip::FinishBuilding() {
+  JoinBuild();
+  VSG_HIP(hipStreamSynchronize(stream_));
+}
 
 void DenseGraphHip::EnsureScratch(size_t n) {
   if (n <= scratch_edges_) return;
@@ -325,6 +362,7 @@
 void DenseGraphHip::SegmentLists(int min_region_size, bool force_constraints, int pass) {
   VSG_REQUIRE(num_frames_ >= 1, -3, "no frames");
   VSG_REQUIRE(!halo_pending_, -3, "the labels of the previous chunk have not been imported");
+  JoinBuild();
   min_region_size_ = min_region_size;
   const int L = (int)lists_.size();
   const size_t N = wh_ * (size_t)num_frames_;
@@ -1732,6 +1770,7 @@
 void DenseGraphHip::CopySpatialBuckets(int t, uint16_t* out) {
   VSG_REQUIRE(t >= 0 && t < num_frames_ && lists_[2 * t].used, -1, "no spatial list for slice");
   ListBuf& lb = lists_[2 * t];
+  JoinBuild();
   std::vector<uint32_t> slots(lb.n);
   std::vector<int32_t> offs(kBucketSlots);
   D2H(slots.data(), lb.slots.get(), (size_t)lb.n, stream_);
diff --git a/video_segment_amd/csrc/dense_graph.h b/video_segment_amd/csrc/dense_graph.h
--- a/video_segment_amd/csrc/dense_graph.h
+++ b/video_segment_amd/csrc/dense_graph.h
@@ -48,11 +48,14 @@
   int num_frames() const { return num_frames_; }
   hipStream_t stream() const { return stream_; }
   hipStream_t aux_stream() const { return aux_stream_; }
+  hipStream_t build_stream() const { return aux2_stream_; }
+  void JoinBuild();
+  int lists_on_side_stream() const { return lists_on_side_; }
 
   void Reset(int max_frames);
   void ForgetLearned();
 
-  void AddFrame(const float* feat_planar_dev, const int32_t* cons_dev);
+  void AddFrame(const float* feat_planar_dev, const int32_t* cons_dev, hipEvent_t planes_ready = nullptr);
   void AddVirtualFrame(const int32_t* ids_dev, int max_label);
   void AddVirtualFrameDeferred();
   void SetHaloLabels(const int32_t* virtual_ids_dev, const int32_t* constrained_ids_dev,
@@ -95,7 +98,12 @@
   void EnsureScratch(size_t n_edges_max);
   void EnsureActiveScratch(size_t n_active_max);
   void DebugHash(const char* where);
-  void SortList(ListBuf& lb, int per_px);
+  struct BuildScratch {
+    uint16_t* keys;
+    int32_t *hist, *sums;
+    hipStream_t stream;
+  };
+  void SortList(ListBuf& lb, int per_px, const BuildScratch& bs);
   void MergeConstrainedHostAssisted();
   NodeArrays nodes() {
     return NodeArrays{parent_.get(), desc_sz_.get(), cons_.get(), flags_.get(), hub8_.get()};
@@ -137,6 +145,13 @@
   std::vector<int32_t> bucket_base_host_;
   DevBuf<uint16_t> keys_tmp_;
   DevBuf<int32_t> hist_tmp_, hist_sums_;
+  DevBuf<uint16_t> keys_side_;
+  DevBuf<int32_t> hist_side_, sums_side_;
+  int build_streams_ = 2;
+  hipEvent_t build_fork_ = nullptr, build_join_ = nullptr;
+  bool side_pending_ = false;
+  bool side_forked_ = false;
+  int lists_on_side_ = 0;
   DevBuf<int32_t> first_label_scratch_;
   DevBuf<int32_t> e_ra_, e_rb_;
   DevBuf<uint32_t> e_gpos_;
diff --git a/video_segment_amd/csrc/device_graph.h b/video_segment_amd/csrc/device_graph.h
--- a/video_segment_amd/csrc/device_graph.h
+++ b/video_segment_amd/csrc/device_graph.h
@@ -58,8 +58,8 @@
                          hipStream_t s);
 void LaunchInterleavedToPlanar(const float* in, size_t n, float* planes, hipStream_t s);
 void LaunchPlanarToInterleaved(const float* planes, size_t n, float* out, hipStream_t s);
-size_t EdgeSortHistInts(size_t n_px);
-size_t EdgeSortSumInts(size_t n_px);
+size_t EdgeSortHistInts(size_t n_px, int per_px = 9);
+size_t EdgeSortSumInts(size_t n_px, int per_px = 9);
 void LaunchSpatialKeys(const float* feat, int W, int H, int l1, uint16_t* keys, int32_t* hist,
                        hipStream_t s);
 void LaunchTemporalKeys(const float* cur, const float* prev, const float* flow, int W, int H,
@@ -169,8 +169,7 @@
   int64_t pool_fallbacks[4], top_level_fallbacks, nested_fallbacks;
   int64_t assumption_reruns, limit_bucket_moves, low_bucket_failures[2], low_bucket_skips[2];
   int64_t zero_pool_flips;
-  int64_t windows_run, rle_stages, wide_launches, group_stages, sorts_hand, sorts_library;
-};
+  int64_t windows_run, rle_stages, wide_launches, group_stages, sorts_hand, sorts_library;};
 struct MergeScratch {
   int active_cap;
   std::function<bool(long long need)> grow_active;
diff --git a/video_segment_amd/csrc/edge_sort.hip b/video_segment_amd/csrc/edge_sort.hip
--- a/video_segment_amd/csrc/edge_sort.hip
+++ b/video_segment_amd/csrc/edge_sort.hip
@@ -283,9 +283,9 @@
   const int tile = per_px == 4 ? kTilePxSpatial : kTilePxTemporal;
   return (int)((n_px + tile - 1) / tile);
 }
-size_t EdgeSortHistInts(size_t n_px) { return (size_t)kBucketSlots * NumTiles(n_px, 9); }
-size_t EdgeSortSumInts(size_t n_px) {
-  return (EdgeSortHistInts(n_px) + kScanPerBlock - 1) / kScanPerBlock;
+size_t EdgeSortHistInts(size_t n_px, int per_px) { return (size_t)kBucketSlots * NumTiles(n_px, per_px); }
+size_t EdgeSortSumInts(size_t n_px, int per_px) {
+  return (EdgeSortHistInts(n_px, per_px) + kScanPerBlock - 1) / kScanPerBlock;
 }
 
 void LaunchSpatialKeys(const float* feat, int W, int H, int l1, uint16_t* keys, int32_t* hist,
diff --git a/video_segment_amd/csrc/stream.cpp b/video_segment_amd/csrc/stream.cpp
--- a/video_segment_amd/csrc/stream.cpp
+++ b/video_segment_amd/csrc/stream.cpp
@@ -159,12 +159,14 @@
   if (bgr) {
     VSG_REQUIRE(stride >= (size_t)W_ * 3, -1, "stride smaller than a row");
     struct InputDrain {
-      hipStream_t s;
+      hipStream_t s, side;
       bool armed = true;
       ~InputDrain() {
-        if (armed) (void)hipStreamSynchronize(s);
-      }
-    } drain{input_stream_};
+        if (!armed) return;
+        (void)hipStreamSynchronize(s);
+        (void)hipStreamSynchronize(side);
+      }
+    } drain{input_stream_, graph_->build_stream()};
     const uint8_t* bgr_dev = bgr;
     if (mem == VSG_MEM_HOST) {
       staging_bgr_.ensure(stride * (size_t)H_);
@@ -218,13 +220,14 @@
       pending_import_ = false;
     } else {
       feature_buffer_.push_back(feat);
-      graph_->AddFrame(feat->get(), nullptr);
+      graph_->AddFrame(feat->get(), nullptr, input_done_);
       if (feature_buffer_.size() > 1) {
         const float* fl = flow_dev_buffer_.empty() ? nullptr : flow_dev_buffer_.back()->get();
         graph_->AddTemporal(feature_buffer_.end()[-1]->get(), feature_buffer_.end()[-2]->get(), fl,
                             false);
       }
     }
+    graph_->JoinBuild();
     VSG_HIP(hipEventRecord(edge_ev_[(size_t)ev + 1], stream_));
     } catch (...) {
       edge_ev_used_ = ev;
@@ -268,6 +271,7 @@
   graph_->AddFrame(feature_buffer_[1]->get(), cons_ids_dev);
   const float* fl = flow_dev_buffer_.empty() ? nullptr : flow_dev_buffer_[1]->get();
   graph_->AddTemporal(nullptr, nullptr, fl, true);
+  graph_->JoinBuild();
 }
 
 void DenseSegmentationHip::ChunkBoundaryOutput(bool flush) {
@@ -296,6 +300,7 @@
     for (const auto& f : flow_dev_buffer_) flows.push_back(f ? f->get() : nullptr);
   }
   graph_->FinishBuilding();
+  build_paths_.lists_on_side_stream = graph_->lists_on_side_stream();
   for (int k = 0; k + 1 < edge_ev_used_; k += 2) {
     float ms = 0;
     VSG_HIP(hipEventElapsedTime(&ms, edge_ev_[(size_t)k], edge_ev_[(size_t)k + 1]));
diff --git a/video_segment_amd/csrc/stream.h b/video_segment_amd/csrc/stream.h
--- a/video_segment_amd/csrc/stream.h
+++ b/video_segment_amd/csrc/stream.h
@@ -88,6 +88,7 @@
   const vsg_timings& last_timings() const { return last_timings_; }
   const GraphTimings& last_graph_timings() const { return last_graph_timings_; }
   const vsg_boundary_paths& last_boundary_paths() const { return boundary_paths_; }
+  const vsg_build_paths& last_build_paths() const { return build_paths_; }
   void CopyLastSmoothed(float* out_interleaved_host);
   int W() const { return W_; }
   int H() const { return H_; }
@@ -155,6 +156,7 @@
   vsg_timings last_timings_;
   GraphTimings last_graph_timings_;
   vsg_boundary_paths boundary_paths_ = {0};
+  vsg_build_paths build_paths_ = {0};
   vsg_timings accum_;
 };
 
diff --git a/video_segment_amd/dense_segmentation.py b/video_segment_amd/dense_segmentation.py
--- a/video_segment_amd/dense_segmentation.py
+++ b/video_segment_amd/dense_segmentation.py
@@ -3,7 +3,7 @@
 import numpy as np
 
 from . import _lib
-from ._lib import (VsgBoundaryPaths, VsgDiagnostics, VsgMergePaths, VsgOptions, VsgSpinePaths, VsgTimings, check,
+from ._lib import (VsgBoundaryPaths, VsgBuildPaths, VsgDiagnostics, VsgMergePaths, VsgOptions, VsgSpinePaths, VsgTimings, check,
                    lib)
 
 
@@ -148,6 +148,11 @@
         check(lib().vsg_stream_last_boundary_paths(self.h, C.byref(m)))
         return m.as_dict()
 
+    def last_build_paths(self):
+        m = VsgBuildPaths()
+        check(lib().vsg_stream_last_build_paths(self.h, C.byref(m)))
+        return m.as_dict()
+
     def last_spine_paths(self):
         m = VsgSpinePaths()
         check(lib().vsg_stream_last_spine_paths(self.h, C.byref(m)))
```

Result: no change. 215.1, median of 3 (+1.2%).
